# louislung/DAE_RNN_News_Recommendation

Hardware: NVIDIA H100
Metric: articles/sec (higher is better)
Workload: dtype f32

## Files before the change

dae_rnn_news_recommendation_b200/csrc/gemm_tc.cu:

```cuda
#include <cuda.h>
#include <cuda_bf16.h>
#include <type_traits>
#include "common.cuh"
#include "topk.cuh"

namespace dae {

constexpr int BLOCK_M = 128;
constexpr int BLOCK_K = 64;
constexpr int WGMMA_K = 16;
constexpr int kThreads = 384;
constexpr int kDecodeN = 128;

__device__ __forceinline__ uint32_t smem_u32(const void* p) { return (uint32_t)__cvta_generic_to_shared(p); }

__device__ __forceinline__ void mbar_init(uint64_t* bar, uint32_t count) {
  asm volatile("mbarrier.init.shared::cta.b64 [%0], %1;" ::"r"(smem_u32(bar)), "r"(count));
}
__device__ __forceinline__ void mbar_expect_tx(uint64_t* bar, uint32_t bytes) {
  asm volatile("mbarrier.arrive.expect_tx.shared::cta.b64 _, [%0], %1;" ::"r"(smem_u32(bar)), "r"(bytes) : "memory");
}
__device__ __forceinline__ void mbar_arrive(uint64_t* bar) {
  asm volatile("mbarrier.arrive.shared::cta.b64 _, [%0];" ::"r"(smem_u32(bar)) : "memory");
}
__device__ __forceinline__ bool mbar_try_wait(uint64_t* bar, uint32_t parity) {
  uint32_t ok;
  asm volatile(
      "{\n"
      ".reg .pred p;\n"
      "mbarrier.try_wait.parity.shared::cta.b64 p, [%1], %2;\n"
      "selp.u32 %0, 1, 0, p;\n"
      "}\n"
      : "=r"(ok)
      : "r"(smem_u32(bar)), "r"(parity)
      : "memory");
  return ok != 0;
}
__device__ __forceinline__ void mbar_wait(uint64_t* bar, uint32_t parity) {
  uint32_t spins = 0;
  while (!mbar_try_wait(bar, parity)) {
    if (++spins > 4096u) {
      __nanosleep(64);
      if (spins > (1u << 26)) __trap();
    }
  }
}
__device__ __forceinline__ void fence_barrier_init() { asm volatile("fence.mbarrier_init.release.cluster;" ::: "memory"); }

__device__ __forceinline__ void tma_load_2d(const CUtensorMap* map, uint64_t* bar, void* dst, int c0, int c1) {
  asm volatile(
      "cp.async.bulk.tensor.2d.shared::cluster.global.mbarrier::complete_tx::bytes [%0], [%1, {%3, %4}], [%2];" ::"r"(smem_u32(dst)),
      "l"(map), "r"(smem_u32(bar)), "r"(c0), "r"(c1)
      : "memory");
}
__device__ __forceinline__ uint32_t cluster_ctarank() { uint32_t r; asm volatile("mov.u32 %0, %%cluster_ctarank;" : "=r"(r)); return r; }
__device__ __forceinline__ void cluster_sync_all() {
  asm volatile("barrier.cluster.arrive.release.aligned;" ::: "memory");
  asm volatile("barrier.cluster.wait.acquire.aligned;" ::: "memory");
}
__device__ __forceinline__ void tma_load_2d_mc(const CUtensorMap* map, uint64_t* bar, void* dst, int c0, int c1, uint16_t cta_mask) {
  asm volatile(
      "cp.async.bulk.tensor.2d.shared::cluster.global.mbarrier::complete_tx::bytes.multicast::cluster [%0], [%1, {%3, %4}], [%2], %5;" ::"r"(
          smem_u32(dst)),
      "l"(map), "r"(smem_u32(bar)), "r"(c0), "r"(c1), "h"(cta_mask)
      : "memory");
}
__device__ __forceinline__ void mbar_arrive_cluster(uint64_t* bar, uint32_t rank) {
  uint32_t raddr;
  asm volatile("mapa.shared::cluster.u32 %0, %1, %2;" : "=r"(raddr) : "r"(smem_u32(bar)), "r"(rank));
  asm volatile("mbarrier.arrive.release.cluster.shared::cluster.b64 _, [%0];" ::"r"(raddr) : "memory");
}
__device__ __forceinline__ void mbar_wait_cluster(uint64_t* bar, uint32_t parity) {
  uint32_t spins = 0;
  for (;;) {
    uint32_t ok;
    asm volatile(
        "{\n"
        ".reg .pred p;\n"
        "mbarrier.try_wait.parity.acquire.cluster.shared::cta.b64 p, [%1], %2;\n"
        "selp.u32 %0, 1, 0, p;\n"
        "}\n"
        : "=r"(ok)
        : "r"(smem_u32(bar)), "r"(parity)
        : "memory");
    if (ok) return;
    if (++spins > 4096u) { __nanosleep(64); if (spins > (1u << 26)) __trap(); }
  }
}

__device__ __forceinline__ void prefetch_tmap(const CUtensorMap* map) {
  asm volatile("prefetch.tensormap [%0];" ::"l"(map) : "memory");
}
__device__ __forceinline__ void named_bar_sync(int id, int threads) { asm volatile("bar.sync %0, %1;" ::"r"(id), "r"(threads) : "memory"); }

__device__ __forceinline__ void wgmma_fence() { asm volatile("wgmma.fence.sync.aligned;" ::: "memory"); }
__device__ __forceinline__ void wgmma_commit() { asm volatile("wgmma.commit_group.sync.aligned;" ::: "memory"); }
template <int N>
__device__ __forceinline__ void wgmma_wait() { asm volatile("wgmma.wait_group.sync.aligned %0;" ::"n"(N) : "memory"); }

__device__ __forceinline__ uint64_t make_desc(uint32_t saddr, uint32_t lbo_bytes, uint32_t sbo_bytes, uint32_t layout = 1) {
  uint64_t d = 0;
  d |= (uint64_t)((saddr >> 4) & 0x3FFF);
  d |= (uint64_t)((lbo_bytes >> 4) & 0x3FFF) << 16;
  d |= (uint64_t)((sbo_bytes >> 4) & 0x3FFF) << 32;
  d |= (uint64_t)layout << 62;
  return d;
}


template <int TA, int TB>
__device__ __forceinline__ void wgmma_n128(float (&d)[64], uint64_t da, uint64_t db, uint32_t scale_d) {
  asm volatile(
      "{\n"
      ".reg .pred p;\n"
      "setp.ne.b32 p, %66, 0;\n"
      "wgmma.mma_async.sync.aligned.m64n128k16.f32.bf16.bf16 "
      "{%0, %1, %2, %3, %4, %5, %6, %7, %8, %9, %10, %11, %12, %13, %14, %15, %16, %17, %18, %19, %20, %21, %22, %23, %24, %25, %26, %27, %28, %29, %30, %31, %32, %33, %34, %35, %36, %37, %38, %39, %40, %41, %42, %43, %44, %45, %46, %47, %48, %49, %50, %51, %52, %53, %54, %55, %56, %57, %58, %59, %60, %61, %62, %63}, %64, %65, p, 1, 1, %67, %68;\n"
      "}\n"
      : "+f"(d[0]), "+f"(d[1]), "+f"(d[2]), "+f"(d[3]), "+f"(d[4]), "+f"(d[5]), "+f"(d[6]), "+f"(d[7]), "+f"(d[8]), "+f"(d[9]), "+f"(d[10]), "+f"(d[11]), "+f"(d[12]), "+f"(d[13]), "+f"(d[14]), "+f"(d[15]), "+f"(d[16]), "+f"(d[17]), "+f"(d[18]), "+f"(d[19]), "+f"(d[20]), "+f"(d[21]), "+f"(d[22]), "+f"(d[23]), "+f"(d[24]), "+f"(d[25]), "+f"(d[26]), "+f"(d[27]), "+f"(d[28]), "+f"(d[29]), "+f"(d[30]), "+f"(d[31]), "+f"(d[32]), "+f"(d[33]), "+f"(d[34]), "+f"(d[35]), "+f"(d[36]), "+f"(d[37]), "+f"(d[38]), "+f"(d[39]), "+f"(d[40]), "+f"(d[41]), "+f"(d[42]), "+f"(d[43]), "+f"(d[44]), "+f"(d[45]), "+f"(d[46]), "+f"(d[47]), "+f"(d[48]), "+f"(d[49]), "+f"(d[50]), "+f"(d[51]), "+f"(d[52]), "+f"(d[53]), "+f"(d[54]), "+f"(d[55]), "+f"(d[56]), "+f"(d[57]), "+f"(d[58]), "+f"(d[59]), "+f"(d[60]), "+f"(d[61]), "+f"(d[62]), "+f"(d[63])
      : "l"(da), "l"(db), "r"(scale_d), "n"(TA), "n"(TB));
}

template <int TA, int TB>
__device__ __forceinline__ void wgmma_n64(float (&d)[32], uint64_t da, uint64_t db, uint32_t scale_d) {
  asm volatile(
      "{\n"
      ".reg .pred p;\n"
      "setp.ne.b32 p, %34, 0;\n"
      "wgmma.mma_async.sync.aligned.m64n64k16.f32.bf16.bf16 "
      "{%0, %1, %2, %3, %4, %5, %6, %7, %8, %9, %10, %11, %12, %13, %14, %15, %16, %17, %18, %19, %20, %21, %22, %23, %24, %25, %26, %27, %28, %29, %30, %31}, %32, %33, p, 1, 1, %35, %36;\n"
      "}\n"
      : "+f"(d[0]), "+f"(d[1]), "+f"(d[2]), "+f"(d[3]), "+f"(d[4]), "+f"(d[5]), "+f"(d[6]), "+f"(d[7]), "+f"(d[8]), "+f"(d[9]), "+f"(d[10]), "+f"(d[11]), "+f"(d[12]), "+f"(d[13]), "+f"(d[14]), "+f"(d[15]), "+f"(d[16]), "+f"(d[17]), "+f"(d[18]), "+f"(d[19]), "+f"(d[20]), "+f"(d[21]), "+f"(d[22]), "+f"(d[23]), "+f"(d[24]), "+f"(d[25]), "+f"(d[26]), "+f"(d[27]), "+f"(d[28]), "+f"(d[29]), "+f"(d[30]), "+f"(d[31])
      : "l"(da), "l"(db), "r"(scale_d), "n"(TA), "n"(TB));
}

struct GemmParams {
  int M, N, K;
  int k_splits;
  int stream_k;
  int atomic;
  int a_mn, b_mn;
  int a_sym_kb;
  float alpha;
  float* C;
  int64_t ldc;
  int n_store;
  int special_col;
  float* special_out;
  const int64_t* indptr; const int32_t* indices; const float* values; const int32_t* rows;
  const float* bv; const float* weight; const double* stats;
  __nv_bfloat16* dz_hi; __nv_bfloat16* dz_lo; int64_t ld_dz;
  float* row_loss_part;
  const int32_t* tile_ptr;
};

struct Sched {
  int tiles_m, tiles, kb_total, kb_per_split, n_work, stream, w, n_cta;
  long long u, u_end;
  __device__ __forceinline__ void init(const GemmParams& p, int block_n, int pair = 0, int block_k = BLOCK_K) {
    const int cta = pair ? (int)(blockIdx.x >> 1) : (int)blockIdx.x;
    n_cta = pair ? (int)(gridDim.x >> 1) : (int)gridDim.x;
    tiles_m = (p.M + BLOCK_M - 1) / BLOCK_M;
    if (pair) tiles_m = (tiles_m + 1) / 2;
    tiles = tiles_m * ((p.N + block_n - 1) / block_n);
    kb_total = (p.K + block_k - 1) / block_k;
    stream = p.stream_k;
    kb_per_split = (kb_total + p.k_splits - 1) / p.k_splits;
    n_work = tiles * p.k_splits;
    w = cta;
    const long long U = (long long)tiles * kb_total;
    u = (long long)cta * U / n_cta;
    u_end = (long long)(cta + 1) * U / n_cta;
  }
  __device__ __forceinline__ bool next(int& mb, int& nb, int& kb0, int& kb1) {
    int tile;
    if (stream) {
      if (u >= u_end) return false;
      tile = (int)(u / kb_total);
      kb0 = (int)(u - (long long)tile * kb_total);
      const long long left = u_end - u;
      kb1 = (left < (long long)(kb_total - kb0)) ? kb0 + (int)left : kb_total;
      u += kb1 - kb0;
    } else {
      if (w >= n_work) return false;
      tile = w % tiles;
      kb0 = (w / tiles) * kb_per_split;
      kb1 = min(kb_total, kb0 + kb_per_split);
      w += n_cta;
    }
    mb = tile % tiles_m;
    nb = tile / tiles_m;
    return true;
  }
};

__device__ __forceinline__ uint32_t pack_bf16(float a, float b) {
  const __nv_bfloat162 v = __floats2bfloat162_rn(a, b);
  return *reinterpret_cast<const uint32_t*>(&v);
}
__device__ __forceinline__ float f_rcp(float x) { float r; asm("rcp.approx.ftz.f32 %0, %1;" : "=f"(r) : "f"(x)); return r; }
__device__ __forceinline__ float f_lg2(float x) { float r; asm("lg2.approx.ftz.f32 %0, %1;" : "=f"(r) : "f"(x)); return r; }
__device__ __forceinline__ float f_ex2(float x) { float r; asm("ex2.approx.ftz.f32 %0, %1;" : "=f"(r) : "f"(x)); return r; }
constexpr float kLog2e = 1.4426950408889634f;

template <int ACT>
__device__ __forceinline__ float act_fast(float z) {
  if (ACT == DAE_ACT_SIGMOID) return f_rcp(1.0f + f_ex2(-kLog2e * z));
  if (ACT == DAE_ACT_TANH) return 1.0f - 2.0f * f_rcp(1.0f + f_ex2(2.0f * kLog2e * z));
  return z;
}


__device__ __forceinline__ float select16(const uint32_t (&r)[16], int j) {
  uint32_t v = r[0];
#pragma unroll
  for (int k = 1; k < 16; ++k) v = (j == k) ? r[k] : v;
  return __uint_as_float(v);
}

template <int ACT, int LOSS>
__device__ __forceinline__ void decode_chunk_generic(const uint32_t (&r)[16], const float* __restrict__ bias, float sc, bool edge,
                                                     int n_lim, int nc, uint32_t (&hpk)[8], uint32_t (&lpk)[8], float& lsum) {
#pragma unroll
  for (int j2 = 0; j2 < 8; ++j2) {
    float dzp[2];
#pragma unroll
    for (int e = 0; e < 2; ++e) {
      const int j = 2 * j2 + e;
      const float z = __uint_as_float(r[j]) + bias[j];
      const float d = act_fast<ACT>(z);
      float dz, lt;
      if (LOSS == DAE_LOSS_CE) {
        const float omd = 1.0f - d;
        const float b = omd + kEps;
        lt = -f_lg2(b);
        dz = (ACT == DAE_ACT_SIGMOID) ? ((omd != 0.0f) ? sc * d : 0.0f) : sc * act_grad_from_y<ACT>(d) * f_rcp(b);
      } else {
        lt = d * d;
        dz = 2.0f * sc * d * act_grad_from_y<ACT>(d);
      }
      if (edge) { const bool in = (nc + j < n_lim); lt = in ? lt : 0.0f; dz = in ? dz : 0.0f; }
      lsum += lt;
      dzp[e] = dz;
    }
    const uint32_t hp = pack_bf16(dzp[0], dzp[1]);
    hpk[j2] = hp;
    lpk[j2] = pack_bf16(dzp[0] - __uint_as_float(hp << 16), dzp[1] - __uint_as_float(hp & 0xffff0000u));
  }
}

__device__ __forceinline__ bool decode_chunk_sigmoid_ce(const uint32_t (&r)[16], const float* __restrict__ biasc, float sc,
                                                        uint32_t (&hpk)[8], uint32_t (&lpk)[8], float& lsum) {
  bool ok = true;
#pragma unroll
  for (int g = 0; g < 4; ++g) {
    float t[4], a[4];
#pragma unroll
    for (int j = 0; j < 4; ++j) {
      t[j] = f_ex2(fmaf(__uint_as_float(r[4 * g + j]), kLog2e, biasc[4 * g + j]));
      a[j] = 1.0f + t[j];
    }
    const float p01 = a[0] * a[1], p23 = a[2] * a[3], P = p01 * p23;
    ok = ok && (P <= 22026.0f);
    const float Rs = f_rcp(P) * sc;
    lsum += f_lg2(P);
    const float r23 = Rs * p23, r01 = Rs * p01;
    const float dz0 = t[0] * (r23 * a[1]), dz1 = t[1] * (r23 * a[0]), dz2 = t[2] * (r01 * a[3]), dz3 = t[3] * (r01 * a[2]);
    const uint32_t h0 = pack_bf16(dz0, dz1), h1 = pack_bf16(dz2, dz3);
    hpk[2 * g] = h0; hpk[2 * g + 1] = h1;
    lpk[2 * g] = pack_bf16(dz0 - __uint_as_float(h0 << 16), dz1 - __uint_as_float(h0 & 0xffff0000u));
    lpk[2 * g + 1] = pack_bf16(dz2 - __uint_as_float(h1 << 16), dz3 - __uint_as_float(h1 & 0xffff0000u));
  }
  return ok;
}

template <int BLOCK_N, int TA, int TB, int BK = BLOCK_K>
__device__ __forceinline__ void mma_kblock(float (&acc)[BLOCK_N / 2], uint32_t sa_hi, uint32_t sa_lo, uint32_t sb_hi, uint32_t sb_lo,
                                           bool first) {
  static_assert(BK == 64 || BK == 32, "k-blocks are 32 or 64 wide");
  constexpr uint32_t kmaj_layout = BK == 64 ? 1u : 2u, kmaj_sbo = BK == 64 ? 1024u : 512u, mn_lbo = 64u * BK * 2u;
  constexpr uint32_t a_layout = TA ? 1u : kmaj_layout, b_layout = TB ? 1u : kmaj_layout;
  constexpr uint32_t a_sbo = TA ? 1024u : kmaj_sbo, b_sbo = TB ? 1024u : kmaj_sbo;
  constexpr uint32_t a_lbo = TA ? mn_lbo : 16u, b_lbo = TB ? mn_lbo : 16u;
  constexpr uint32_t a_step = TA ? 2048u : 32u, b_step = TB ? 2048u : 32u;
#pragma unroll
  for (int k = 0; k < BK / WGMMA_K; ++k) {
    const uint64_t da_hi = make_desc(sa_hi + k * a_step, a_lbo, a_sbo, a_layout), da_lo = make_desc(sa_lo + k * a_step, a_lbo, a_sbo, a_layout);
    const uint64_t db_hi = make_desc(sb_hi + k * b_step, b_lbo, b_sbo, b_layout), db_lo = make_desc(sb_lo + k * b_step, b_lbo, b_sbo, b_layout);
    const uint32_t sc = (first && k == 0) ? 0u : 1u;
    if constexpr (BLOCK_N == 128) {
      wgmma_n128<TA, TB>(acc, da_lo, db_hi, sc);
      wgmma_n128<TA, TB>(acc, da_hi, db_lo, 1u);
      wgmma_n128<TA, TB>(acc, da_hi, db_hi, 1u);
    } else {
      wgmma_n64<TA, TB>(acc, da_lo, db_hi, sc);
      wgmma_n64<TA, TB>(acc, da_hi, db_lo, 1u);
      wgmma_n64<TA, TB>(acc, da_hi, db_hi, 1u);
    }
  }
}

__device__ __forceinline__ void stage_ld16(const float* src, uint32_t (&r)[16]) {
#pragma unroll
  for (int q = 0; q < 4; ++q) {
    const float4 v = reinterpret_cast<const float4*>(src)[q];
    r[4 * q] = __float_as_uint(v.x); r[4 * q + 1] = __float_as_uint(v.y); r[4 * q + 2] = __float_as_uint(v.z); r[4 * q + 3] = __float_as_uint(v.w);
  }
}


template <int BLOCK_N, int STAGES, int PAIR, int BK = BLOCK_K, class SchedT>
__device__ __forceinline__ void tma_produce(const GemmParams& p, SchedT& sched, uint8_t* smem, uint64_t* full_bar, uint64_t* empty_bar,
                                            uint32_t crank, const CUtensorMap* tm_a_hi, const CUtensorMap* tm_a_lo,
                                            const CUtensorMap* tm_b_hi, const CUtensorMap* tm_b_lo, const CUtensorMap* tm_at_hi,
                                            const CUtensorMap* tm_at_lo) {
  constexpr int A_TILE = BLOCK_M * BK * 2;
  constexpr int B_TILE = BLOCK_N * BK * 2;
  constexpr int STAGE_BYTES = 2 * A_TILE + 2 * B_TILE;
  int stage = 0; uint32_t phase = 0;
  int mb, nb, kb0, kb1;
  while (sched.next(mb, nb, kb0, kb1)) {
    for (int kb = kb0; kb < kb1; ++kb) {
      if (PAIR) mbar_wait_cluster(&empty_bar[stage], phase ^ 1); else mbar_wait(&empty_bar[stage], phase ^ 1);
      uint8_t* sa_hi = smem + stage * STAGE_BYTES;
      uint8_t* sa_lo = sa_hi + A_TILE;
      uint8_t* sb_hi = sa_lo + A_TILE;
      uint8_t* sb_lo = sb_hi + B_TILE;
      const int mt = PAIR ? mb * 2 + (int)crank : mb;
      mbar_expect_tx(&full_bar[stage], STAGE_BYTES);
      if (p.a_sym_kb > 0 && kb >= p.a_sym_kb) {
#pragma unroll
        for (int j = 0; j < BLOCK_M / 64; ++j) {
          tma_load_2d(tm_at_hi, &full_bar[stage], sa_hi + j * (64 * BK * 2), mt * BLOCK_M + j * 64, (kb - p.a_sym_kb) * BK);
          tma_load_2d(tm_at_lo, &full_bar[stage], sa_lo + j * (64 * BK * 2), mt * BLOCK_M + j * 64, (kb - p.a_sym_kb) * BK);
        }
      } else if (!p.a_mn) {
        tma_load_2d(tm_a_hi, &full_bar[stage], sa_hi, kb * BK, mt * BLOCK_M);
        tma_load_2d(tm_a_lo, &full_bar[stage], sa_lo, kb * BK, mt * BLOCK_M);
      } else {
#pragma unroll
        for (int j = 0; j < BLOCK_M / 64; ++j) {
          tma_load_2d(tm_a_hi, &full_bar[stage], sa_hi + j * (64 * BK * 2), mt * BLOCK_M + j * 64, kb * BK);
          tma_load_2d(tm_a_lo, &full_bar[stage], sa_lo + j * (64 * BK * 2), mt * BLOCK_M + j * 64, kb * BK);
        }
      }
      const int kbb = (p.a_sym_kb > 0 && kb >= p.a_sym_kb) ? kb - p.a_sym_kb : kb;
      if (PAIR) {
        const int off = (int)crank * 8192, n_half = nb * BLOCK_N + (int)crank * 64;
        if (!p.b_mn) {
          tma_load_2d_mc(tm_b_hi, &full_bar[stage], sb_hi + off, kbb * BK, n_half, 0x3);
          tma_load_2d_mc(tm_b_lo, &full_bar[stage], sb_lo + off, kbb * BK, n_half, 0x3);
        } else {
          tma_load_2d_mc(tm_b_hi, &full_bar[stage], sb_hi + off, n_half, kbb * BK, 0x3);
          tma_load_2d_mc(tm_b_lo, &full_bar[stage], sb_lo + off, n_half, kbb * BK, 0x3);
        }
      } else if (!p.b_mn) {
        tma_load_2d(tm_b_hi, &full_bar[stage], sb_hi, kbb * BK, nb * BLOCK_N);
        tma_load_2d(tm_b_lo, &full_bar[stage], sb_lo, kbb * BK, nb * BLOCK_N);
      } else {
#pragma unroll
        for (int j = 0; j < BLOCK_N / 64; ++j) {
          tma_load_2d(tm_b_hi, &full_bar[stage], sb_hi + j * (64 * BK * 2), nb * BLOCK_N + j * 64, kbb * BK);
          tma_load_2d(tm_b_lo, &full_bar[stage], sb_lo + j * (64 * BK * 2), nb * BLOCK_N + j * 64, kbb * BK);
        }
      }
      if (++stage == STAGES) { stage = 0; phase ^= 1; }
    }
  }
}

template <int BLOCK_N, int STAGES, int PAIR, int MAJ, int BK = BLOCK_K>
__device__ __forceinline__ void mma_work_item(float (&acc)[BLOCK_N / 2], const GemmParams& p, uint8_t* smem, uint64_t* full_bar,
                                              uint64_t* empty_bar, int wg, int lane, uint32_t crank, int& stage, uint32_t& phase,
                                              int kb0, int kb1) {
  constexpr int A_TILE = BLOCK_M * BK * 2;
  constexpr int B_TILE = BLOCK_N * BK * 2;
  constexpr int STAGE_BYTES = 2 * A_TILE + 2 * B_TILE;
  auto release = [&](int s) {
    __syncwarp();
    if (lane == 0) { mbar_arrive(&empty_bar[s]); if (PAIR) mbar_arrive_cluster(&empty_bar[s], crank ^ 1u); }
  };
  int prev = -1;
  auto run_k = [&](auto ta, auto tb, int kb_begin, int kb_end) {
    for (int kb = kb_begin; kb < kb_end; ++kb) {
      mbar_wait(&full_bar[stage], phase);
      const uint32_t sa_hi = smem_u32(smem + stage * STAGE_BYTES) + wg * (64 * BK * 2);
      const uint32_t sa_lo = sa_hi + A_TILE;
      const uint32_t sb_hi = smem_u32(smem + stage * STAGE_BYTES) + 2 * A_TILE, sb_lo = sb_hi + B_TILE;
      wgmma_fence();
      mma_kblock<BLOCK_N, decltype(ta)::value, decltype(tb)::value, BK>(acc, sa_hi, sa_lo, sb_hi, sb_lo, kb == kb0);
      wgmma_commit();
      wgmma_wait<1>();
      if (prev >= 0) release(prev);
      prev = stage;
      if (++stage == STAGES) { stage = 0; phase ^= 1; }
    }
  };
  using K0 = std::integral_constant<int, 0>;
  using K1 = std::integral_constant<int, 1>;
  if constexpr ((MAJ & 4) != 0) {
    run_k(K0{}, K1{}, kb0, min(kb1, p.a_sym_kb));
    run_k(K1{}, K1{}, max(kb0, p.a_sym_kb), kb1);
  } else {
    run_k(std::integral_constant<int, MAJ & 1>{}, std::integral_constant<int, (MAJ >> 1) & 1>{}, kb0, kb1);
  }
  wgmma_wait<0>();
  if (prev >= 0) release(prev);
}

template <int BLOCK_N, int STAGES, int PAIR, int MAJ, int BK = BLOCK_K>
__global__ void __launch_bounds__(kThreads, 1) gemm_bf16x3_kernel(const __grid_constant__ CUtensorMap tm_a_hi,
                                                                   const __grid_constant__ CUtensorMap tm_a_lo,
                                                                   const __grid_constant__ CUtensorMap tm_b_hi,
                                                                   const __grid_constant__ CUtensorMap tm_b_lo,
                                                                   const __grid_constant__ CUtensorMap tm_at_hi,
                                                                   const __grid_constant__ CUtensorMap tm_at_lo,
                                                                   const GemmParams p) {
  static_assert(!PAIR || BLOCK_N == 128, "CTA pairs split the B tile into two 64-row halves");
  constexpr int STAGE_BYTES = 2 * BLOCK_M * BK * 2 + 2 * BLOCK_N * BK * 2;
  constexpr int SROW = BLOCK_N + 4;
  constexpr int kParts = 2;
  constexpr int HALF_N = BLOCK_N / kParts;
  extern __shared__ __align__(1024) uint8_t smem_raw[];
  uint8_t* smem = reinterpret_cast<uint8_t*>((reinterpret_cast<uintptr_t>(smem_raw) + 1023) & ~(uintptr_t)1023);
  float* stg = reinterpret_cast<float*>(smem + STAGES * STAGE_BYTES);
  __shared__ __align__(8) uint64_t full_bar[STAGES], empty_bar[STAGES];

  const int warp = threadIdx.x >> 5, lane = threadIdx.x & 31;
  Sched sched;
  sched.init(p, BLOCK_N, PAIR, BK);
  const uint32_t crank = PAIR ? cluster_ctarank() : 0u;

  if (warp == 0 && lane == 0) {
    prefetch_tmap(&tm_a_hi); prefetch_tmap(&tm_a_lo); prefetch_tmap(&tm_b_hi); prefetch_tmap(&tm_b_lo);
    if (p.a_sym_kb > 0) { prefetch_tmap(&tm_at_hi); prefetch_tmap(&tm_at_lo); }
  }
  if (warp == 1 && lane == 0) {
    for (int s = 0; s < STAGES; ++s) { mbar_init(&full_bar[s], 1); mbar_init(&empty_bar[s], PAIR ? 16 : 8); }
    fence_barrier_init();
  }
  if (PAIR) cluster_sync_all(); else __syncthreads();

  if (warp == 0) {
    if (lane == 0)
      tma_produce<BLOCK_N, STAGES, PAIR, BK>(p, sched, smem, full_bar, empty_bar, crank, &tm_a_hi, &tm_a_lo, &tm_b_hi, &tm_b_lo, &tm_at_hi,
                                         &tm_at_lo);
  } else if (warp >= 4) {
    const int wg = (warp >> 2) - 1;
    const int wi = warp & 3;
    const int quarter = wg * 2 + (wi & 1);
    const int half = wi >> 1;
    float acc[BLOCK_N / 2];
#pragma unroll
    for (int i = 0; i < BLOCK_N / 2; ++i) acc[i] = 0.0f;
    int stage = 0; uint32_t phase = 0;
    int mb, nb, kb0, kb1;
    while (sched.next(mb, nb, kb0, kb1)) {
      if (PAIR) mb = mb * 2 + (int)crank;
      mma_work_item<BLOCK_N, STAGES, PAIR, MAJ, BK>(acc, p, smem, full_bar, empty_bar, wg, lane, crank, stage, phase, kb0, kb1);

      named_bar_sync(1 + wg, 128);
      {
        const int r0 = wg * 64 + wi * 16 + (lane >> 2), c0 = 2 * (lane & 3);
#pragma unroll
        for (int j = 0; j < BLOCK_N / 8; ++j) {
          *reinterpret_cast<float2*>(&stg[r0 * SROW + 8 * j + c0]) = make_float2(acc[4 * j], acc[4 * j + 1]);
          *reinterpret_cast<float2*>(&stg[(r0 + 8) * SROW + 8 * j + c0]) = make_float2(acc[4 * j + 2], acc[4 * j + 3]);
        }
      }
      named_bar_sync(1 + wg, 128);
      const int n0 = nb * BLOCK_N + half * HALF_N;
      const float* tr = stg + (quarter * 32) * SROW + half * HALF_N;
      const int m_base = mb * BLOCK_M + quarter * 32;
      const bool vec_ok = ((p.ldc & 3) == 0) && ((reinterpret_cast<uintptr_t>(p.C) & 15) == 0);
#pragma unroll 1
      for (int c = 0; c < HALF_N / 16; ++c) {
        const int nc = n0 + c * 16;
        const bool interior = vec_ok && (m_base + 32 <= p.M) && (nc + 16 <= p.n_store) && (p.special_col < nc || p.special_col >= nc + 16);
        if (interior) {
          const int rsub = lane >> 2, c4 = (lane & 3) * 4;
          float* dst = p.C + (int64_t)(m_base + rsub) * p.ldc + nc + c4;
          const int64_t step = 8 * p.ldc;
#pragma unroll
          for (int i = 0; i < 4; ++i) {
            float4 v = *reinterpret_cast<const float4*>(&tr[(rsub + 8 * i) * SROW + c * 16 + c4]);
            v.x *= p.alpha; v.y *= p.alpha; v.z *= p.alpha; v.w *= p.alpha;
            if (p.atomic) atomicAdd(reinterpret_cast<float4*>(dst), v); else *reinterpret_cast<float4*>(dst) = v;
            dst += step;
          }
        } else {
          const int rsub = lane >> 4, csub = lane & 15;
          const int n = nc + csub;
          for (int i = 0; i < 16; ++i) {
            const int rr = 2 * i + rsub;
            const int mm = m_base + rr;
            const float v = p.alpha * tr[rr * SROW + c * 16 + csub];
            if (mm < p.M) {
              if (n == p.special_col) {
                if (p.atomic) atomicAdd(p.special_out + mm, v); else p.special_out[mm] = v;
              } else if (n < p.n_store) {
                float* dst = p.C + (int64_t)mm * p.ldc + n;
                if (p.atomic) atomicAdd(dst, v); else *dst = v;
              }
            }
          }
        }
      }
    }
  }

  if (PAIR) cluster_sync_all();
}

constexpr int kDecodeThreads = 640;
constexpr int kDecodeBK = 32;
constexpr int kDecodeStages = 4;
constexpr int kRegsProducer = 32, kRegsMma = 104, kRegsEpilogue = 120;
static_assert(128 * kRegsProducer + 256 * kRegsMma + 256 * kRegsEpilogue <= kDecodeThreads * 96, "register budget");

template <int R> __device__ __forceinline__ void regs_dec() { asm volatile("setmaxnreg.dec.sync.aligned.u32 %0;" ::"n"(R)); }
template <int R> __device__ __forceinline__ void regs_inc() { asm volatile("setmaxnreg.inc.sync.aligned.u32 %0;" ::"n"(R)); }

template <int ACT, int LOSS>
__global__ void __launch_bounds__(kDecodeThreads, 1) decode_fused_kernel(const __grid_constant__ CUtensorMap tm_a_hi,
                                                                         const __grid_constant__ CUtensorMap tm_a_lo,
                                                                         const __grid_constant__ CUtensorMap tm_b_hi,
                                                                         const __grid_constant__ CUtensorMap tm_b_lo,
                                                                         const GemmParams p) {
  constexpr int BLOCK_N = kDecodeN, STAGES = kDecodeStages, BK = kDecodeBK;
  constexpr int STAGE_BYTES = 2 * BLOCK_M * BK * 2 + 2 * BLOCK_N * BK * 2;
  constexpr int SROW = BLOCK_N + 4;
  constexpr int kParts = 2;
  constexpr int HALF_N = BLOCK_N / kParts;
  constexpr bool kFast = (ACT == DAE_ACT_SIGMOID) && (LOSS == DAE_LOSS_CE);
  extern __shared__ __align__(1024) uint8_t smem_raw[];
  uint8_t* smem = reinterpret_cast<uint8_t*>((reinterpret_cast<uintptr_t>(smem_raw) + 1023) & ~(uintptr_t)1023);
  float* stg = reinterpret_cast<float*>(smem + STAGES * STAGE_BYTES);
  __shared__ __align__(8) uint64_t full_bar[STAGES], empty_bar[STAGES], staged_bar[2], drained_bar[2];
  __shared__ float s_bias[2][BLOCK_N];
  __shared__ float s_biasc[kFast ? 2 : 1][kFast ? BLOCK_N : 1];
  __shared__ __align__(16) uint8_t s_stage[8][2][32][48];

  const int warp = threadIdx.x >> 5, lane = threadIdx.x & 31;
  const int role = warp >> 2;
  Sched sched;

  if (warp == 0 && lane == 0) { prefetch_tmap(&tm_a_hi); prefetch_tmap(&tm_a_lo); prefetch_tmap(&tm_b_hi); prefetch_tmap(&tm_b_lo); }
  if (warp == 1 && lane == 0) {
    for (int s = 0; s < STAGES; ++s) { mbar_init(&full_bar[s], 1); mbar_init(&empty_bar[s], 8); }
    for (int h = 0; h < 2; ++h) { mbar_init(&staged_bar[h], 4); mbar_init(&drained_bar[h], 4); }
    fence_barrier_init();
  }
  __syncthreads();

  if (role == 0) {
    regs_dec<kRegsProducer>();
    sched.init(p, BLOCK_N, 0, BK);
    if (warp == 0 && lane == 0)
      tma_produce<BLOCK_N, STAGES, 0, BK>(p, sched, smem, full_bar, empty_bar, 0u, &tm_a_hi, &tm_a_lo, &tm_b_hi, &tm_b_lo, &tm_a_hi, &tm_a_lo);
  } else if (role <= 2) {
    regs_inc<kRegsMma>();
    sched.init(p, BLOCK_N, 0, BK);
    const int h = role - 1;
    const int wi = warp & 3;
    float acc[BLOCK_N / 2];
#pragma unroll
    for (int i = 0; i < BLOCK_N / 2; ++i) acc[i] = 0.0f;
    int stage = 0; uint32_t phase = 0, tphase = 0;
    int mb, nb, kb0, kb1;
    while (sched.next(mb, nb, kb0, kb1)) {
      mma_work_item<BLOCK_N, STAGES, 0, 0, BK>(acc, p, smem, full_bar, empty_bar, h, lane, 0u, stage, phase, kb0, kb1);
      mbar_wait(&drained_bar[h], tphase ^ 1);
      const int r0 = h * 64 + wi * 16 + (lane >> 2), c0 = 2 * (lane & 3);
#pragma unroll
      for (int j = 0; j < BLOCK_N / 8; ++j) {
        *reinterpret_cast<float2*>(&stg[r0 * SROW + 8 * j + c0]) = make_float2(acc[4 * j], acc[4 * j + 1]);
        *reinterpret_cast<float2*>(&stg[(r0 + 8) * SROW + 8 * j + c0]) = make_float2(acc[4 * j + 2], acc[4 * j + 3]);
      }
      __syncwarp();
      if (lane == 0) mbar_arrive(&staged_bar[h]);
      tphase ^= 1;
    }
  } else {
    regs_inc<kRegsEpilogue>();
    sched.init(p, BLOCK_N, 0, BK);
    const int h = role - 3;
    const int ew = warp - 12;
    const int wi = warp & 3;
    const int quarter = h * 2 + (wi & 1);
    const int half = wi >> 1;
    const int row_in_tile = quarter * 32 + lane;
    const int tid = threadIdx.x - 128 * role;
    const int tiles_n = (p.N + BLOCK_N - 1) / BLOCK_N;
    uint8_t* stg_hi = reinterpret_cast<uint8_t*>(&s_stage[ew][0][0][0]);
    uint8_t* stg_lo = reinterpret_cast<uint8_t*>(&s_stage[ew][1][0][0]);
    const int rsub = lane >> 1, csub = lane & 1;
    uint32_t tphase = 0;
    int mb, nb, kb0, kb1;
    while (sched.next(mb, nb, kb0, kb1)) {
      const float* srow = stg + row_in_tile * SROW + half * HALF_N;
      const int m = mb * BLOCK_M + row_in_tile;
      const int n0 = nb * BLOCK_N + half * HALF_N;
      int64_t pc = 0, pe = 0;
      int c0 = 0x7fffffff, c1 = 0x7fffffff, c2 = 0x7fffffff;
      float v0 = 0.0f, v1 = 0.0f, v2 = 0.0f;
      float sc = 0.0f;
      if (m < p.M) {
        const int64_t row = p.rows ? (int64_t)p.rows[m] : (int64_t)m;
        const int64_t rbeg = p.indptr[row];
        const int32_t* tp = p.tile_ptr + (int64_t)m * (kParts * tiles_n + 1) + nb * kParts + half;
        pc = rbeg + tp[0]; pe = rbeg + tp[1];
        if (pc < pe) { c0 = p.indices[pc]; v0 = p.values[pc]; }
        if (pc + 1 < pe) { c1 = p.indices[pc + 1]; v1 = p.values[pc + 1]; }
        if (pc + 2 < pe) { c2 = p.indices[pc + 2]; v2 = p.values[pc + 2]; }
        sc = (p.weight ? p.weight[m] : 1.0f) / ((float)p.stats[DAE_STAT_SUM_W] + kEps);
      }
      named_bar_sync(1 + h, 128);
      {
        const float b = (nb * BLOCK_N + tid < p.N) ? p.bv[nb * BLOCK_N + tid] : 0.0f;
        s_bias[h][tid] = b;
        if (kFast) s_biasc[h][tid] = b * kLog2e;
      }
      mbar_wait(&staged_bar[h], tphase);
      named_bar_sync(1 + h, 128);
      const float inv_sc = (sc != 0.0f) ? 1.0f / sc : 0.0f;
      const bool edge = (n0 + HALF_N > p.N);
      float lsum = 0.0f;
      const int m_base = mb * BLOCK_M + quarter * 32;
      const int n_lim = edge ? p.N : 0x7fffffff;
#pragma unroll 1
      for (int c = 0; c < HALF_N / 16; ++c) {
        uint32_t r[16];
        stage_ld16(srow + c * 16, r);
        const int nc = n0 + c * 16;
        if (m < p.M) {
          const float* bias = &s_bias[h][half * HALF_N + c * 16];
          uint32_t hpk[8], lpk[8];
          bool fast_ok = false;
          if (kFast && !edge) {
            const float l0 = lsum;
            fast_ok = decode_chunk_sigmoid_ce(r, &s_biasc[h][half * HALF_N + c * 16], sc, hpk, lpk, lsum);
            if (!fast_ok) { lsum = l0; decode_chunk_generic<ACT, LOSS>(r, bias, sc, edge, n_lim, nc, hpk, lpk, lsum); }
          } else {
            decode_chunk_generic<ACT, LOSS>(r, bias, sc, edge, n_lim, nc, hpk, lpk, lsum);
          }
          uint4* sh = reinterpret_cast<uint4*>(stg_hi + lane * 48);
          uint4* sl = reinterpret_cast<uint4*>(stg_lo + lane * 48);
          sh[0] = make_uint4(hpk[0], hpk[1], hpk[2], hpk[3]); sh[1] = make_uint4(hpk[4], hpk[5], hpk[6], hpk[7]);
          sl[0] = make_uint4(lpk[0], lpk[1], lpk[2], lpk[3]); sl[1] = make_uint4(lpk[4], lpk[5], lpk[6], lpk[7]);
          while (c0 < nc + 16) {
            const float x = v0;
            const int j = c0 - nc;
            __nv_bfloat16* ph = reinterpret_cast<__nv_bfloat16*>(stg_hi + lane * 48) + j;
            __nv_bfloat16* pl = reinterpret_cast<__nv_bfloat16*>(stg_lo + lane * 48) + j;
            float d;
            if (kFast && fast_ok && sc != 0.0f) d = (__bfloat162float(*ph) + __bfloat162float(*pl)) * inv_sc;
            else d = act_fast<ACT>(select16(r, j) + bias[j]);
            const float gp = act_grad_from_y<ACT>(d);
            float dz;
            if (LOSS == DAE_LOSS_CE) {
              const float a = d + kEps, b = (1.0f - d) + kEps;
              const float la = f_lg2(a), lb = f_lg2(b);
              lsum += lb - (x * la + (1.0f - x) * lb);
              dz = sc * gp * ((1.0f - x) * f_rcp(b) - x * f_rcp(a));
            } else {
              const float e2 = x - d;
              lsum += e2 * e2 - d * d;
              dz = -2.0f * sc * e2 * gp;
            }
            const __nv_bfloat16 hb = __float2bfloat16_rn(dz);
            *ph = hb;
            *pl = __float2bfloat16_rn(dz - __bfloat162float(hb));
            ++pc;
            c0 = c1; v0 = v1; c1 = c2; v1 = v2;
            c2 = 0x7fffffff;
            if (pc + 2 < pe) { c2 = p.indices[pc + 2]; v2 = p.values[pc + 2]; }
          }
        }
        __syncwarp();
        if (nc < p.ld_dz) {
#pragma unroll
          for (int i = 0; i < 2; ++i) {
            const int rr = rsub + 16 * i;
            if (m_base + rr < p.M) {
              const int64_t off = (int64_t)(m_base + rr) * p.ld_dz + nc + csub * 8;
              *reinterpret_cast<uint4*>(p.dz_hi + off) = *reinterpret_cast<const uint4*>(stg_hi + rr * 48 + csub * 16);
              *reinterpret_cast<uint4*>(p.dz_lo + off) = *reinterpret_cast<const uint4*>(stg_lo + rr * 48 + csub * 16);
            }
          }
        }
        __syncwarp();
      }
      if (lane == 0) mbar_arrive(&drained_bar[h]);
      tphase ^= 1;
      if (m < p.M) atomicAdd(p.row_loss_part + m, (LOSS == DAE_LOSS_CE) ? lsum * 0.6931471805599453f : lsum);
    }
  }
}

constexpr int kTopkMaxK = 32;
constexpr int kTopkMaxSplits = 32;
constexpr int kTopkMinTiles = 4;
constexpr int kTopkBK = 64;
constexpr int kTopkStages = 2;

struct TopkParams {
  GemmParams g;
  int k, splits;
  int exclude;
  int64_t diag_offset;
  float* ws_val; int32_t* ws_idx;
};

struct TopkSched {
  int tiles_n, splits, kb_total, n_work, n_cta, w;
  int mb, split, t, t_end;
  bool first, last;
  __device__ __forceinline__ void init(const TopkParams& tp, int block_n, int block_k) {
    const int tiles_m = (tp.g.M + BLOCK_M - 1) / BLOCK_M;
    tiles_n = (tp.g.N + block_n - 1) / block_n;
    splits = tp.splits;
    kb_total = (tp.g.K + block_k - 1) / block_k;
    n_work = tiles_m * splits;
    n_cta = (int)gridDim.x;
    w = (int)blockIdx.x - n_cta;
    mb = split = t = t_end = 0;
    first = last = false;
  }
  __device__ __forceinline__ bool next(int& mb_, int& nb, int& kb0, int& kb1) {
    first = false;
    if (t >= t_end) {
      w += n_cta;
      if (w >= n_work) return false;
      mb = w / splits;
      split = w - mb * splits;
      t = split * tiles_n / splits;
      t_end = (split + 1) * tiles_n / splits;
      first = true;
    }
    mb_ = mb; nb = t; kb0 = 0; kb1 = kb_total;
    last = (++t == t_end);
    return true;
  }
};

template <int KMAX>
__device__ __forceinline__ void topk_offer(float (&sv)[KMAX], int (&si)[KMAX], float& thr, int k, float v, int col, int n_lim,
                                           int excl) {
  if (!(v > thr) || col >= n_lim || col == excl) return;
#pragma unroll
  for (int j = KMAX - 1; j >= 0; --j) {
    const bool up = (j > 0) && (v > sv[j > 0 ? j - 1 : 0]);
    const bool here = v > sv[j];
    si[j] = up ? si[j > 0 ? j - 1 : 0] : (here ? col : si[j]);
    sv[j] = up ? sv[j > 0 ? j - 1 : 0] : (here ? v : sv[j]);
  }
  float t = sv[0];
#pragma unroll
  for (int j = 1; j < KMAX; ++j)
    asm("{\n.reg .pred q;\nsetp.eq.s32 q, %1, %2;\nselp.f32 %0, %3, %0, q;\n}\n" : "+f"(t) : "r"(j), "r"(k - 1), "f"(sv[j]));
  thr = t;
}

template <int KMAX>
__global__ void __launch_bounds__(kDecodeThreads, 1) topk_kernel(const __grid_constant__ CUtensorMap tm_a_hi,
                                                                 const __grid_constant__ CUtensorMap tm_a_lo,
                                                                 const __grid_constant__ CUtensorMap tm_b_hi,
                                                                 const __grid_constant__ CUtensorMap tm_b_lo,
                                                                 const TopkParams tp) {
  constexpr int BLOCK_N = kDecodeN, STAGES = kTopkStages, BK = kTopkBK;
  constexpr int STAGE_BYTES = 2 * BLOCK_M * BK * 2 + 2 * BLOCK_N * BK * 2;
  constexpr int SROW = BLOCK_N + 4;
  constexpr int HALF_N = BLOCK_N / 2;
  const GemmParams& p = tp.g;
  extern __shared__ __align__(1024) uint8_t smem_raw[];
  uint8_t* smem = reinterpret_cast<uint8_t*>((reinterpret_cast<uintptr_t>(smem_raw) + 1023) & ~(uintptr_t)1023);
  float* stg = reinterpret_cast<float*>(smem + STAGES * STAGE_BYTES);
  __shared__ __align__(8) uint64_t full_bar[STAGES], empty_bar[STAGES], staged_bar[2], drained_bar[2];

  const int warp = threadIdx.x >> 5, lane = threadIdx.x & 31;
  const int role = warp >> 2;
  TopkSched sched;

  if (warp == 0 && lane == 0) { prefetch_tmap(&tm_a_hi); prefetch_tmap(&tm_a_lo); prefetch_tmap(&tm_b_hi); prefetch_tmap(&tm_b_lo); }
  if (warp == 1 && lane == 0) {
    for (int s = 0; s < STAGES; ++s) { mbar_init(&full_bar[s], 1); mbar_init(&empty_bar[s], 8); }
    for (int h = 0; h < 2; ++h) { mbar_init(&staged_bar[h], 4); mbar_init(&drained_bar[h], 4); }
    fence_barrier_init();
  }
  __syncthreads();

  if (role == 0) {
    regs_dec<kRegsProducer>();
    sched.init(tp, BLOCK_N, BK);
    if (warp == 0 && lane == 0)
      tma_produce<BLOCK_N, STAGES, 0, BK>(p, sched, smem, full_bar, empty_bar, 0u, &tm_a_hi, &tm_a_lo, &tm_b_hi, &tm_b_lo, &tm_a_hi, &tm_a_lo);
  } else if (role <= 2) {
    regs_inc<kRegsMma>();
    sched.init(tp, BLOCK_N, BK);
    const int h = role - 1;
    const int wi = warp & 3;
    float acc[BLOCK_N / 2];
#pragma unroll
    for (int i = 0; i < BLOCK_N / 2; ++i) acc[i] = 0.0f;
    int stage = 0; uint32_t phase = 0, tphase = 0;
    int mb, nb, kb0, kb1;
    while (sched.next(mb, nb, kb0, kb1)) {
      mma_work_item<BLOCK_N, STAGES, 0, 0, BK>(acc, p, smem, full_bar, empty_bar, h, lane, 0u, stage, phase, kb0, kb1);
      mbar_wait(&drained_bar[h], tphase ^ 1);
      const int r0 = h * 64 + wi * 16 + (lane >> 2), c0 = 2 * (lane & 3);
#pragma unroll
      for (int j = 0; j < BLOCK_N / 8; ++j) {
        *reinterpret_cast<float2*>(&stg[r0 * SROW + 8 * j + c0]) = make_float2(acc[4 * j], acc[4 * j + 1]);
        *reinterpret_cast<float2*>(&stg[(r0 + 8) * SROW + 8 * j + c0]) = make_float2(acc[4 * j + 2], acc[4 * j + 3]);
      }
      __syncwarp();
      if (lane == 0) mbar_arrive(&staged_bar[h]);
      tphase ^= 1;
    }
  } else {
    regs_inc<kRegsEpilogue>();
    sched.init(tp, BLOCK_N, BK);
    const int h = role - 3;
    const int wi = warp & 3;
    const int quarter = h * 2 + (wi & 1);
    const int half = wi >> 1;
    const int row_in_tile = quarter * 32 + lane;
    const int k = tp.k;
    const float* srow = stg + row_in_tile * SROW + half * HALF_N;
    float sv[KMAX];
    int si[KMAX];
    float thr = neg_inf();
    int m = 0, excl = -1;
    uint32_t tphase = 0;
    int mb, nb, kb0, kb1;
    while (sched.next(mb, nb, kb0, kb1)) {
      if (sched.first) {
#pragma unroll
        for (int j = 0; j < KMAX; ++j) { sv[j] = neg_inf(); si[j] = -1; }
        thr = neg_inf();
        m = mb * BLOCK_M + row_in_tile;
        const int64_t e = (int64_t)m + tp.diag_offset;
        excl = (tp.exclude && e >= 0 && e < p.N) ? (int)e : -1;
      }
      const int n0 = nb * BLOCK_N + half * HALF_N;
      mbar_wait(&staged_bar[h], tphase);
      if (m < p.M) {
#pragma unroll 1
        for (int c = 0; c < HALF_N; c += 4) {
          const float4 v = *reinterpret_cast<const float4*>(srow + c);
          if (fmaxf(fmaxf(v.x, v.y), fmaxf(v.z, v.w)) > thr) {
            topk_offer<KMAX>(sv, si, thr, k, v.x, n0 + c, p.N, excl);
            topk_offer<KMAX>(sv, si, thr, k, v.y, n0 + c + 1, p.N, excl);
            topk_offer<KMAX>(sv, si, thr, k, v.z, n0 + c + 2, p.N, excl);
            topk_offer<KMAX>(sv, si, thr, k, v.w, n0 + c + 3, p.N, excl);
          }
        }
      }
      __syncwarp();
      if (lane == 0) mbar_arrive(&drained_bar[h]);
      tphase ^= 1;
      if (sched.last && m < p.M) {
        const int64_t base = ((int64_t)m * (2 * sched.splits) + 2 * sched.split + half) * k;
#pragma unroll
        for (int j = 0; j < KMAX; ++j)
          if (j < k) { tp.ws_val[base + j] = sv[j]; tp.ws_idx[base + j] = si[j]; }
      }
    }
  }
}

__global__ void decode_tile_ptr_kernel(const int64_t* __restrict__ indptr, const int32_t* __restrict__ indices,
                                       const int32_t* __restrict__ rows, int M, int n_half_tiles, int half_n,
                                       int32_t* __restrict__ tile_ptr) {
  const int t = blockIdx.x * blockDim.x + threadIdx.x;
  const int m = blockIdx.y;
  if (t > n_half_tiles || m >= M) return;
  const int64_t row = rows ? (int64_t)rows[m] : (int64_t)m;
  const int64_t b = indptr[row], e = indptr[row + 1];
  const int target = t * half_n;
  int64_t lo = b, hi = e;
  while (lo < hi) { const int64_t mid = (lo + hi) >> 1; if (indices[mid] < target) lo = mid + 1; else hi = mid; }
  tile_ptr[(int64_t)m * (n_half_tiles + 1) + t] = (int32_t)(lo - b);
}

__global__ void split_bf16_kernel(const float* __restrict__ src, int rows, int cols, int64_t ld_src, __nv_bfloat16* __restrict__ hi,
                                  __nv_bfloat16* __restrict__ lo, int64_t ld_dst, int ones_col, float scale) {
  const int64_t total = (int64_t)rows * ld_dst;
  for (int64_t i = (int64_t)blockIdx.x * blockDim.x + threadIdx.x; i < total; i += (int64_t)gridDim.x * blockDim.x) {
    const int64_t r = i / ld_dst;
    const int c = (int)(i - r * ld_dst);
    float v = (c < cols) ? src[r * ld_src + c] * scale : 0.0f;
    if (c == ones_col) v = 1.0f;
    const __nv_bfloat16 h = __float2bfloat16_rn(v);
    hi[i] = h;
    lo[i] = __float2bfloat16_rn(v - __bfloat162float(h));
  }
}

__global__ void sym_split_kernel(const float* __restrict__ G, int B, int64_t ldg, float alpha, __nv_bfloat16* __restrict__ hi,
                                 __nv_bfloat16* __restrict__ lo, int64_t ld) {
  __shared__ float t[32][33];
  const int bx = blockIdx.x * 32, by = blockIdx.y * 32;
  const int tx = threadIdx.x, ty = threadIdx.y;
  for (int j = ty; j < 32; j += 8) {
    const int r = bx + j, c = by + tx;
    t[j][tx] = (r < B && c < B) ? G[(int64_t)r * ldg + c] : 0.0f;
  }
  __syncthreads();
  for (int j = ty; j < 32; j += 8) {
    const int r = by + j, c = bx + tx;
    if (r < B && c < ld) {
      float v = 0.0f;
      if (c < B) v = alpha * (G[(int64_t)r * ldg + c] + t[tx][j]);
      const __nv_bfloat16 h = __float2bfloat16_rn(v);
      hi[(int64_t)r * ld + c] = h;
      lo[(int64_t)r * ld + c] = __float2bfloat16_rn(v - __bfloat162float(h));
    }
  }
}

typedef CUresult (*PFN_encodeTiled)(CUtensorMap*, CUtensorMapDataType, cuuint32_t, void*, const cuuint64_t*, const cuuint64_t*,
                                    const cuuint32_t*, const cuuint32_t*, CUtensorMapInterleave, CUtensorMapSwizzle,
                                    CUtensorMapL2promotion, CUtensorMapFloatOOBfill);

static PFN_encodeTiled get_encode() {
  static PFN_encodeTiled fn = nullptr;
  if (!fn) {
    void* sym = nullptr;
    cudaDriverEntryPointQueryResult q;
    if (cudaGetDriverEntryPoint("cuTensorMapEncodeTiled", &sym, cudaEnableDefault, &q) == cudaSuccess && q == cudaDriverEntryPointSuccess)
      fn = reinterpret_cast<PFN_encodeTiled>(sym);
  }
  return fn;
}

static int make_map(CUtensorMap* m, const void* base, uint64_t inner, uint64_t outer, uint64_t ld, uint32_t box_outer,
                    uint32_t box_inner = 64) {
  PFN_encodeTiled enc = get_encode();
  if (!enc) { set_error("cuTensorMapEncodeTiled entry point not found"); return DAE_ERR_CUDA; }
  cuuint64_t dims[2] = {inner, outer};
  cuuint64_t strides[1] = {ld * 2};
  cuuint32_t box[2] = {box_inner, box_outer};
  cuuint32_t estr[2] = {1, 1};
  CUresult r = enc(m, CU_TENSOR_MAP_DATA_TYPE_BFLOAT16, 2, const_cast<void*>(base), dims, strides, box, estr,
                   CU_TENSOR_MAP_INTERLEAVE_NONE, box_inner == 64 ? CU_TENSOR_MAP_SWIZZLE_128B : CU_TENSOR_MAP_SWIZZLE_64B,
                   CU_TENSOR_MAP_L2_PROMOTION_L2_256B,
                   CU_TENSOR_MAP_FLOAT_OOB_FILL_NONE);
  if (r != CUDA_SUCCESS) { set_error("cuTensorMapEncodeTiled failed (%d): inner=%llu outer=%llu ld=%llu", (int)r,
                                     (unsigned long long)inner, (unsigned long long)outer, (unsigned long long)ld); return DAE_ERR_CUDA; }
  return DAE_OK;
}

struct Operand { const void* hi; const void* lo; int64_t ld; int mn_major; };

template <typename Kern>
static int ensure_smem_attr(Kern kern, int smem, bool (&done)[64]) {
  int dev = 0;
  DAE_CUDA(cudaGetDevice(&dev));
  if (dev < 0 || dev >= 64 || !done[dev]) {
    DAE_CUDA(cudaFuncSetAttribute(kern, cudaFuncAttributeMaxDynamicSharedMemorySize, smem));
    if (dev >= 0 && dev < 64) done[dev] = true;
  }
  return DAE_OK;
}


static int g_pair_mode = -1;
static int g_lean = 0;

template <int BLOCK_N, int STAGES, int PAIR, int MAJ, int BK = BLOCK_K>
static int launch_gemm_maj(const Operand& A, const Operand& B, GemmParams p, cudaStream_t st) {
  CUtensorMap ta_hi, ta_lo, tb_hi, tb_lo;
  int rc;
  constexpr int B_ROWS = PAIR ? BLOCK_N / 2 : BLOCK_N;
  if (!A.mn_major) {
    const uint64_t a_cols = p.a_sym_kb > 0 ? (uint64_t)p.M : (uint64_t)p.K;
    if ((rc = make_map(&ta_hi, A.hi, a_cols, p.M, A.ld, BLOCK_M, BK))) return rc;
    if ((rc = make_map(&ta_lo, A.lo, a_cols, p.M, A.ld, BLOCK_M, BK))) return rc;
  } else {
    if ((rc = make_map(&ta_hi, A.hi, p.M, p.K, A.ld, BK))) return rc;
    if ((rc = make_map(&ta_lo, A.lo, p.M, p.K, A.ld, BK))) return rc;
  }
  if (!B.mn_major) {
    if ((rc = make_map(&tb_hi, B.hi, p.K, p.N, B.ld, B_ROWS, BK))) return rc;
    if ((rc = make_map(&tb_lo, B.lo, p.K, p.N, B.ld, B_ROWS, BK))) return rc;
  } else {
    const uint64_t b_rows = p.a_sym_kb > 0 ? (uint64_t)p.M : (uint64_t)p.K;
    if ((rc = make_map(&tb_hi, B.hi, p.N, b_rows, B.ld, BK))) return rc;
    if ((rc = make_map(&tb_lo, B.lo, p.N, b_rows, B.ld, BK))) return rc;
  }
  p.a_mn = A.mn_major; p.b_mn = B.mn_major;
  CUtensorMap tat_hi = ta_hi, tat_lo = ta_lo;
  if (p.a_sym_kb > 0) {
    if (PAIR || A.mn_major) { set_error("dae_gemm_sym_bf16x3: unsupported configuration"); return DAE_ERR_UNSUPPORTED; }
    if ((rc = make_map(&tat_hi, A.hi, p.M, p.M, A.ld, 64))) return rc;
    if ((rc = make_map(&tat_lo, A.lo, p.M, p.M, A.ld, 64))) return rc;
  }
  constexpr int smem = STAGES * (2 * BLOCK_M * BK * 2 + 2 * BLOCK_N * BK * 2) + BLOCK_M * (BLOCK_N + 4) * 4 + 1024;
  int tiles_m = (p.M + BLOCK_M - 1) / BLOCK_M;
  if (PAIR) tiles_m = (tiles_m + 1) / 2;
  const int tiles_n = (p.N + BLOCK_N - 1) / BLOCK_N;
  const int kblocks = (p.K + BK - 1) / BK;
  auto kern = gemm_bf16x3_kernel<BLOCK_N, STAGES, PAIR, MAJ, BK>;
  static bool attr_done[64] = {false};
  if ((rc = ensure_smem_attr(kern, smem, attr_done))) return rc;
  const int slots = PAIR ? sm_count() / 2 : sm_count();
  int n;
  if (p.stream_k) {
    const long long units = (long long)tiles_m * tiles_n * kblocks;
    long long g = units / (6 * BLOCK_K / BK);
    if (g < 1) g = 1;
    n = (int)(g < slots ? g : slots);
  } else {
    const int items = tiles_m * tiles_n * p.k_splits;
    n = items < slots ? items : slots;
  }
  if (!PAIR) {
    kern<<<n, kThreads, smem, st>>>(ta_hi, ta_lo, tb_hi, tb_lo, tat_hi, tat_lo, p);
  } else {
    cudaLaunchConfig_t cfg{};
    cfg.gridDim = dim3(2 * n); cfg.blockDim = dim3(kThreads); cfg.dynamicSmemBytes = smem; cfg.stream = st;
    cudaLaunchAttribute at[1];
    at[0].id = cudaLaunchAttributeClusterDimension;
    at[0].val.clusterDim.x = 2; at[0].val.clusterDim.y = 1; at[0].val.clusterDim.z = 1;
    cfg.attrs = at; cfg.numAttrs = 1;
    DAE_CUDA(cudaLaunchKernelEx(&cfg, kern, ta_hi, ta_lo, tb_hi, tb_lo, tat_hi, tat_lo, p));
  }
  return DAE_OK;
}

template <int BLOCK_N, int STAGES, int PAIR, int BK = BLOCK_K>
static int launch_gemm(const Operand& A, const Operand& B, GemmParams p, cudaStream_t st) {
  if (!A.mn_major && !B.mn_major) return launch_gemm_maj<BLOCK_N, STAGES, PAIR, 0, BK>(A, B, p, st);
  if (A.mn_major && !B.mn_major) return launch_gemm_maj<BLOCK_N, STAGES, PAIR, 1, BK>(A, B, p, st);
  if (!A.mn_major) return launch_gemm_maj<BLOCK_N, STAGES, PAIR, 2, BK>(A, B, p, st);
  return launch_gemm_maj<BLOCK_N, STAGES, PAIR, 3, BK>(A, B, p, st);
}

template <int ACT, int LOSS>
static int launch_decode(const Operand& A, const Operand& B, const GemmParams& p, cudaStream_t st) {
  CUtensorMap ta_hi, ta_lo, tb_hi, tb_lo;
  int rc;
  if ((rc = make_map(&ta_hi, A.hi, p.K, p.M, A.ld, BLOCK_M, kDecodeBK))) return rc;
  if ((rc = make_map(&ta_lo, A.lo, p.K, p.M, A.ld, BLOCK_M, kDecodeBK))) return rc;
  if ((rc = make_map(&tb_hi, B.hi, p.K, p.N, B.ld, kDecodeN, kDecodeBK))) return rc;
  if ((rc = make_map(&tb_lo, B.lo, p.K, p.N, B.ld, kDecodeN, kDecodeBK))) return rc;
  constexpr int smem = kDecodeStages * (2 * BLOCK_M * kDecodeBK * 2 + 2 * kDecodeN * kDecodeBK * 2) + BLOCK_M * (kDecodeN + 4) * 4 + 1024;
  auto kern = decode_fused_kernel<ACT, LOSS>;
  static bool attr_done[64] = {false};
  if ((rc = ensure_smem_attr(kern, smem, attr_done))) return rc;
  const int tiles = ((p.M + BLOCK_M - 1) / BLOCK_M) * ((p.N + kDecodeN - 1) / kDecodeN);
  const int n = tiles < sm_count() ? tiles : sm_count();
  kern<<<n, kDecodeThreads, smem, st>>>(ta_hi, ta_lo, tb_hi, tb_lo, p);
  return DAE_OK;
}

template <int KMAX>
static int launch_topk(const Operand& A, const Operand& B, const TopkParams& tp, cudaStream_t st) {
  CUtensorMap ta_hi, ta_lo, tb_hi, tb_lo;
  int rc;
  const GemmParams& p = tp.g;
  if ((rc = make_map(&ta_hi, A.hi, p.K, p.M, A.ld, BLOCK_M, kTopkBK))) return rc;
  if ((rc = make_map(&ta_lo, A.lo, p.K, p.M, A.ld, BLOCK_M, kTopkBK))) return rc;
  if ((rc = make_map(&tb_hi, B.hi, p.K, p.N, B.ld, kDecodeN, kTopkBK))) return rc;
  if ((rc = make_map(&tb_lo, B.lo, p.K, p.N, B.ld, kDecodeN, kTopkBK))) return rc;
  constexpr int smem = kTopkStages * (2 * BLOCK_M * kTopkBK * 2 + 2 * kDecodeN * kTopkBK * 2) + BLOCK_M * (kDecodeN + 4) * 4 + 1024;
  auto kern = topk_kernel<KMAX>;
  static bool attr_done[64] = {false};
  if ((rc = ensure_smem_attr(kern, smem, attr_done))) return rc;
  const int items = ((p.M + BLOCK_M - 1) / BLOCK_M) * tp.splits;
  const int n = items < sm_count() ? items : sm_count();
  kern<<<n, kDecodeThreads, smem, st>>>(ta_hi, ta_lo, tb_hi, tb_lo, tp);
  return DAE_OK;
}

static int topk_splits(int n_query, int n_corpus, int requested) {
  const int tiles_m = (n_query + BLOCK_M - 1) / BLOCK_M, tiles_n = (n_corpus + kDecodeN - 1) / kDecodeN;
  int s = requested;
  if (s <= 0) {
    s = (sm_count() + tiles_m - 1) / tiles_m;
    const int by_len = tiles_n / kTopkMinTiles;
    if (s > by_len) s = by_len;
  }
  if (s > tiles_n) s = tiles_n;
  if (s > kTopkMaxSplits) s = kTopkMaxSplits;
  return s < 1 ? 1 : s;
}

static int64_t topk_workspace_bytes(int n_query, int k, int splits) {
  return (int64_t)n_query * 2 * splits * k * (int64_t)(sizeof(float) + sizeof(int32_t));
}

static bool use_pair() { return g_pair_mode == 1 && !g_lean; }

}

using namespace dae;

extern "C" int dae_split_bf16(const float* src, int32_t rows, int32_t cols, int64_t ld_src, void* hi, void* lo, int64_t ld_dst,
                              int32_t ones_col, float scale, void* stream) {
  DAE_REQUIRE(src && hi && lo && rows > 0 && cols > 0 && ld_src >= cols && ld_dst >= cols, "dae_split_bf16: bad arguments");
  const int64_t total = (int64_t)rows * ld_dst;
  const int cap = sm_count() * 16;
  const int blocks = (int)((total + 255) / 256 < cap ? (total + 255) / 256 : cap);
  split_bf16_kernel<<<blocks, 256, 0, (cudaStream_t)stream>>>(src, rows, cols, ld_src, (__nv_bfloat16*)hi, (__nv_bfloat16*)lo, ld_dst,
                                                              ones_col, scale);
  DAE_CHECK_LAUNCH("dae_split_bf16");
  return DAE_OK;
}

extern "C" int dae_sym_split_bf16(const float* G, int32_t B, int64_t ldg, float alpha, void* hi, void* lo, int64_t ld, void* stream) {
  DAE_REQUIRE(G && hi && lo && B > 0 && ldg >= B && ld >= B, "dae_sym_split_bf16: bad arguments");
  dim3 grid((unsigned)((ld + 31) / 32), (B + 31) / 32), block(32, 8);
  sym_split_kernel<<<grid, block, 0, (cudaStream_t)stream>>>(G, B, ldg, alpha, (__nv_bfloat16*)hi, (__nv_bfloat16*)lo, ld);
  DAE_CHECK_LAUNCH("dae_sym_split_bf16");
  return DAE_OK;
}

extern "C" int dae_gemm_config(int32_t pair_mode, int32_t lean) {
  dae::g_pair_mode = pair_mode < 0 ? -1 : (pair_mode ? 1 : 0);
  dae::g_lean = lean ? 1 : 0;
  return DAE_OK;
}

extern "C" int dae_gemm_bf16x3(int32_t M, int32_t N, int32_t K, float alpha, const void* a_hi, const void* a_lo, int64_t lda,
                               int32_t a_mn_major, const void* b_hi, const void* b_lo, int64_t ldb, int32_t b_mn_major, float* C,
                               int64_t ldc, int32_t n_store, int32_t special_col, float* special_out, int32_t k_splits,
                               int32_t accumulate, void* stream) {
  DAE_REQUIRE(a_hi && a_lo && b_hi && b_lo && C && M > 0 && N > 0 && K > 0, "dae_gemm_bf16x3: bad arguments");
  DAE_REQUIRE(lda % 8 == 0 && ldb % 8 == 0, "dae_gemm_bf16x3: operand leading dimensions must be multiples of 8 (TMA 16-byte strides)");
  DAE_REQUIRE(((uintptr_t)a_hi | (uintptr_t)a_lo | (uintptr_t)b_hi | (uintptr_t)b_lo) % 16 == 0, "dae_gemm_bf16x3: operands must be 16-byte aligned");
  cudaStream_t st = (cudaStream_t)stream;
  if (n_store <= 0 || n_store > N) n_store = N;
  const int kblocks = (K + BLOCK_K - 1) / BLOCK_K;
  const int tm = (M + 127) / 128, tn128 = (N + 127) / 128, tn64 = (N + 63) / 64;
  const int sms = sm_count();
  int stream_k = 0;
  if (k_splits < 0) {
    const int t = tm * tn128;
    stream_k = (t % sms == 0) ? 0 : 1;
    k_splits = 1;
  }
  if (k_splits < 1) k_splits = 1;
  if (k_splits > kblocks) k_splits = kblocks;
  {
    const int per = (kblocks + k_splits - 1) / k_splits;
    k_splits = (kblocks + per - 1) / per;
  }
  const bool partial = (k_splits > 1) || stream_k;
  if (partial && !accumulate) {
    DAE_CUDA(cudaMemset2DAsync(C, ldc * sizeof(float), 0, (size_t)n_store * sizeof(float), M, st));
    if (special_col >= 0 && special_out) DAE_CUDA(cudaMemsetAsync(special_out, 0, sizeof(float) * M, st));
  }
  GemmParams p{};
  p.M = M; p.N = N; p.K = K; p.k_splits = k_splits; p.stream_k = stream_k; p.atomic = (partial || accumulate) ? 1 : 0; p.alpha = alpha;
  p.C = C; p.ldc = ldc; p.n_store = n_store;
  p.special_col = (special_out ? special_col : -1); p.special_out = special_out;
  Operand A{a_hi, a_lo, lda, a_mn_major}, B{b_hi, b_lo, ldb, b_mn_major};
  int rc;
  const int tiles128 = tm * tn128 * k_splits, tiles64 = tm * tn64 * k_splits;
  const float cost128 = 2.0f * (float)((tiles128 + sms - 1) / sms), cost64 = 1.1f * (float)((tiles64 + sms - 1) / sms);
  if (g_lean) rc = launch_gemm<64, 2, 0>(A, B, p, st);
  else if (use_pair()) rc = launch_gemm<128, 2, 1>(A, B, p, st);
  else if (stream_k) rc = launch_gemm<128, 4, 0, 32>(A, B, p, st);
  else if (!stream_k && cost64 < cost128) rc = launch_gemm<64, 3, 0>(A, B, p, st);
  else rc = launch_gemm<128, 2, 0>(A, B, p, st);
  if (rc) return rc;
  DAE_CHECK_LAUNCH("dae_gemm_bf16x3");
  return DAE_OK;
}

extern "C" int dae_gemm_sym_bf16x3(int32_t M, int32_t N, float alpha, const void* g_hi, const void* g_lo, int64_t ldg, const void* b_hi,
                                   const void* b_lo, int64_t ldb, float* C, int64_t ldc, int32_t accumulate, void* stream) {
  DAE_REQUIRE(g_hi && g_lo && b_hi && b_lo && C && M > 0 && N > 0, "dae_gemm_sym_bf16x3: bad arguments");
  DAE_REQUIRE(ldg % 8 == 0 && ldb % 8 == 0 && ldg >= M && ldb >= N, "dae_gemm_sym_bf16x3: leading dimensions must be multiples of 8 and cover the matrices");
  DAE_REQUIRE(((uintptr_t)g_hi | (uintptr_t)g_lo | (uintptr_t)b_hi | (uintptr_t)b_lo) % 16 == 0, "dae_gemm_sym_bf16x3: operands must be 16-byte aligned");
  GemmParams p{};
  const int kb_half = (M + BLOCK_K - 1) / BLOCK_K;
  p.M = M; p.N = N; p.K = 2 * kb_half * BLOCK_K; p.k_splits = 1; p.stream_k = 1; p.atomic = 1; p.alpha = alpha;
  p.C = C; p.ldc = ldc; p.n_store = N; p.special_col = -1; p.special_out = nullptr; p.a_sym_kb = kb_half;
  if (!accumulate) DAE_CUDA(cudaMemset2DAsync(C, ldc * sizeof(float), 0, (size_t)N * sizeof(float), M, (cudaStream_t)stream));
  Operand A{g_hi, g_lo, ldg, 0}, B{b_hi, b_lo, ldb, 1};
  int rc = launch_gemm_maj<128, 2, 0, 6>(A, B, p, (cudaStream_t)stream);
  if (rc) return rc;
  DAE_CHECK_LAUNCH("dae_gemm_sym_bf16x3");
  return DAE_OK;
}

extern "C" int dae_decode_prepare(int32_t Brows, int32_t F, const int64_t* indptr, const int32_t* indices, const int32_t* rows,
                                  float* row_loss_part, int32_t* tile_ptr, void* stream) {
  DAE_REQUIRE(Brows > 0 && F > 0 && indptr && indices && row_loss_part && tile_ptr, "dae_decode_prepare: bad arguments");
  cudaStream_t st = (cudaStream_t)stream;
  DAE_CUDA(cudaMemsetAsync(row_loss_part, 0, sizeof(float) * Brows, st));
  const int n_half = 2 * ((F + kDecodeN - 1) / kDecodeN);
  dim3 grid((n_half + 1 + 127) / 128, Brows);
  decode_tile_ptr_kernel<<<grid, 128, 0, st>>>(indptr, indices, rows, Brows, n_half, kDecodeN / 2, tile_ptr);
  DAE_CHECK_LAUNCH("dae_decode_prepare");
  return DAE_OK;
}

extern "C" int dae_decode_fused_bf16x3(int32_t Brows, int32_t F, int32_t K, const void* e_hi, const void* e_lo, int64_t lde,
                                       const void* w_hi, const void* w_lo, int64_t ldw, const int64_t* indptr, const int32_t* indices,
                                       const float* values, const int32_t* rows, const float* bv, int32_t dec_act, int32_t loss_func,
                                       const float* weight, const double* stats, void* dz_hi, void* dz_lo, int64_t ld_dz,
                                       float* row_loss_part, int32_t* tile_ptr, int32_t prepared, void* stream) {
  DAE_REQUIRE(e_hi && e_lo && w_hi && w_lo && indptr && indices && values && bv && stats && dz_hi && dz_lo && row_loss_part && tile_ptr,
              "dae_decode_fused_bf16x3: null pointer");
  DAE_REQUIRE(loss_func == DAE_LOSS_CE || loss_func == DAE_LOSS_MSE, "dae_decode_fused_bf16x3: cosine loss uses the unfused path");
  DAE_REQUIRE(lde % 8 == 0 && ldw % 8 == 0 && ld_dz % 32 == 0 && ld_dz >= F, "dae_decode_fused_bf16x3: bad leading dimensions");
  cudaStream_t st = (cudaStream_t)stream;
  GemmParams p{};
  p.M = Brows; p.N = F; p.K = K; p.k_splits = 1; p.alpha = 1.0f; p.special_col = -1;
  p.indptr = indptr; p.indices = indices; p.values = values; p.rows = rows; p.bv = bv; p.weight = weight; p.stats = stats;
  p.dz_hi = (__nv_bfloat16*)dz_hi; p.dz_lo = (__nv_bfloat16*)dz_lo; p.ld_dz = ld_dz; p.row_loss_part = row_loss_part;
  p.tile_ptr = tile_ptr;
  if (!prepared) {
    int rc0 = dae_decode_prepare(Brows, F, indptr, indices, rows, row_loss_part, tile_ptr, stream);
    if (rc0) return rc0;
  }
  Operand A{e_hi, e_lo, lde, 0}, B{w_hi, w_lo, ldw, 0};
  int rc = 0;
#define DAE_DEC(ACT, LOSS) rc = launch_decode<ACT, LOSS>(A, B, p, st)
  if (loss_func == DAE_LOSS_CE) {
    if (dec_act == DAE_ACT_SIGMOID) DAE_DEC(DAE_ACT_SIGMOID, DAE_LOSS_CE);
    else if (dec_act == DAE_ACT_TANH) DAE_DEC(DAE_ACT_TANH, DAE_LOSS_CE);
    else DAE_DEC(DAE_ACT_NONE, DAE_LOSS_CE);
  } else {
    if (dec_act == DAE_ACT_SIGMOID) DAE_DEC(DAE_ACT_SIGMOID, DAE_LOSS_MSE);
    else if (dec_act == DAE_ACT_TANH) DAE_DEC(DAE_ACT_TANH, DAE_LOSS_MSE);
    else DAE_DEC(DAE_ACT_NONE, DAE_LOSS_MSE);
  }
#undef DAE_DEC
  if (rc) return rc;
  DAE_CHECK_LAUNCH("dae_decode_fused_bf16x3");
  return DAE_OK;
}

extern "C" int dae_similarity_topk_workspace(int32_t n_query, int32_t n_corpus, int32_t k, int32_t splits, int64_t* bytes) {
  DAE_REQUIRE(bytes && n_query > 0 && n_corpus > 0, "dae_similarity_topk_workspace: bad arguments");
  DAE_REQUIRE(k >= 1 && k <= kTopkMaxK, "dae_similarity_topk_workspace: k = %d is outside the supported range 1 <= k <= %d", k, kTopkMaxK);
  *bytes = topk_workspace_bytes(n_query, k, topk_splits(n_query, n_corpus, splits));
  return DAE_OK;
}

extern "C" int dae_similarity_topk_bf16x3(int32_t n_query, int32_t n_corpus, int32_t dim, const void* q_hi, const void* q_lo, int64_t ldq,
                                          const void* c_hi, const void* c_lo, int64_t ldc, int32_t k, int64_t diag_offset, int32_t exclude,
                                          int32_t splits, void* workspace, int64_t workspace_bytes, int32_t* idx_out, float* val_out,
                                          void* stream) {
  DAE_REQUIRE(q_hi && q_lo && c_hi && c_lo && workspace && idx_out && val_out, "dae_similarity_topk_bf16x3: null pointer");
  DAE_REQUIRE(n_query > 0 && n_corpus > 0 && dim > 0, "dae_similarity_topk_bf16x3: bad sizes");
  DAE_REQUIRE(k >= 1 && k <= kTopkMaxK, "dae_similarity_topk_bf16x3: k = %d is outside the supported range 1 <= k <= %d", k, kTopkMaxK);
  DAE_REQUIRE(ldq >= dim && ldc >= dim && ldq % 8 == 0 && ldc % 8 == 0,
              "dae_similarity_topk_bf16x3: leading dimensions must cover dim and be multiples of 8 (TMA 16-byte strides)");
  DAE_REQUIRE(((uintptr_t)q_hi | (uintptr_t)q_lo | (uintptr_t)c_hi | (uintptr_t)c_lo | (uintptr_t)workspace) % 16 == 0,
              "dae_similarity_topk_bf16x3: operands and workspace must be 16-byte aligned");
  const int s = topk_splits(n_query, n_corpus, splits);
  const int64_t need = topk_workspace_bytes(n_query, k, s);
  DAE_REQUIRE(workspace_bytes >= need, "dae_similarity_topk_bf16x3: workspace of %lld bytes, %lld needed (dae_similarity_topk_workspace)",
              (long long)workspace_bytes, (long long)need);
  cudaStream_t st = (cudaStream_t)stream;
  TopkParams tp{};
  tp.g.M = n_query; tp.g.N = n_corpus; tp.g.K = dim; tp.g.k_splits = 1; tp.g.alpha = 1.0f; tp.g.special_col = -1;
  tp.k = k; tp.splits = s; tp.exclude = exclude ? 1 : 0; tp.diag_offset = diag_offset;
  tp.ws_val = reinterpret_cast<float*>(workspace);
  tp.ws_idx = reinterpret_cast<int32_t*>(reinterpret_cast<float*>(workspace) + (int64_t)n_query * 2 * s * k);
  Operand A{q_hi, q_lo, ldq, 0}, B{c_hi, c_lo, ldc, 0};
  int rc = (k <= 16) ? launch_topk<16>(A, B, tp, st) : launch_topk<32>(A, B, tp, st);
  if (rc) return rc;
  DAE_CHECK_LAUNCH("dae_similarity_topk_bf16x3");
  topk_merge_kernel<<<(n_query + 7) / 8, 256, 0, st>>>(tp.ws_val, tp.ws_idx, n_query, 2 * s, k, idx_out, val_out);
  DAE_CHECK_LAUNCH("dae_similarity_topk_bf16x3 (merge)");
  return DAE_OK;
}
```

Before: 2.294 million.

## Transpose fused decode GEMM with 160-wide batch tiles and simplified warp roles

The fused decode kernel now computes the transposed product, with features on the M side and batch rows on the N side, using m64n160k16 wgmma tiles. Warp roles drop from 20 warps with setmaxnreg rebalancing to 14 warps: 8 MMA warps, 5 epilogue warps and 1 TMA producer. Staging moves to a swizzled, column-major shared buffer that is reused in place for the bf16 outputs. This aims for better tensor-core tile shape and fewer barrier and staging round-trips, but it changes tile_ptr semantics, shrinks epilogue parallelism, and leaves one epilogue thread per batch row serially scanning 128 features.

After: 2.340 million, median of 6. 2.0% higher.

```diff
diff --git a/dae_rnn_news_recommendation_b200/csrc/gemm_tc.cu b/dae_rnn_news_recommendation_b200/csrc/gemm_tc.cu
--- a/dae_rnn_news_recommendation_b200/csrc/gemm_tc.cu
+++ b/dae_rnn_news_recommendation_b200/csrc/gemm_tc.cu
@@ -10,7 +10,6 @@
 constexpr int BLOCK_K = 64;
 constexpr int WGMMA_K = 16;
 constexpr int kThreads = 384;
-constexpr int kDecodeN = 128;
 
 __device__ __forceinline__ uint32_t smem_u32(const void* p) { return (uint32_t)__cvta_generic_to_shared(p); }
 
@@ -118,6 +117,19 @@
       "{%0, %1, %2, %3, %4, %5, %6, %7, %8, %9, %10, %11, %12, %13, %14, %15, %16, %17, %18, %19, %20, %21, %22, %23, %24, %25, %26, %27, %28, %29, %30, %31, %32, %33, %34, %35, %36, %37, %38, %39, %40, %41, %42, %43, %44, %45, %46, %47, %48, %49, %50, %51, %52, %53, %54, %55, %56, %57, %58, %59, %60, %61, %62, %63}, %64, %65, p, 1, 1, %67, %68;\n"
       "}\n"
       : "+f"(d[0]), "+f"(d[1]), "+f"(d[2]), "+f"(d[3]), "+f"(d[4]), "+f"(d[5]), "+f"(d[6]), "+f"(d[7]), "+f"(d[8]), "+f"(d[9]), "+f"(d[10]), "+f"(d[11]), "+f"(d[12]), "+f"(d[13]), "+f"(d[14]), "+f"(d[15]), "+f"(d[16]), "+f"(d[17]), "+f"(d[18]), "+f"(d[19]), "+f"(d[20]), "+f"(d[21]), "+f"(d[22]), "+f"(d[23]), "+f"(d[24]), "+f"(d[25]), "+f"(d[26]), "+f"(d[27]), "+f"(d[28]), "+f"(d[29]), "+f"(d[30]), "+f"(d[31]), "+f"(d[32]), "+f"(d[33]), "+f"(d[34]), "+f"(d[35]), "+f"(d[36]), "+f"(d[37]), "+f"(d[38]), "+f"(d[39]), "+f"(d[40]), "+f"(d[41]), "+f"(d[42]), "+f"(d[43]), "+f"(d[44]), "+f"(d[45]), "+f"(d[46]), "+f"(d[47]), "+f"(d[48]), "+f"(d[49]), "+f"(d[50]), "+f"(d[51]), "+f"(d[52]), "+f"(d[53]), "+f"(d[54]), "+f"(d[55]), "+f"(d[56]), "+f"(d[57]), "+f"(d[58]), "+f"(d[59]), "+f"(d[60]), "+f"(d[61]), "+f"(d[62]), "+f"(d[63])
+      : "l"(da), "l"(db), "r"(scale_d), "n"(TA), "n"(TB));
+}
+
+template <int TA, int TB>
+__device__ __forceinline__ void wgmma_n160(float (&d)[80], uint64_t da, uint64_t db, uint32_t scale_d) {
+  asm volatile(
+      "{\n"
+      ".reg .pred p;\n"
+      "setp.ne.b32 p, %82, 0;\n"
+      "wgmma.mma_async.sync.aligned.m64n160k16.f32.bf16.bf16 "
+      "{%0, %1, %2, %3, %4, %5, %6, %7, %8, %9, %10, %11, %12, %13, %14, %15, %16, %17, %18, %19, %20, %21, %22, %23, %24, %25, %26, %27, %28, %29, %30, %31, %32, %33, %34, %35, %36, %37, %38, %39, %40, %41, %42, %43, %44, %45, %46, %47, %48, %49, %50, %51, %52, %53, %54, %55, %56, %57, %58, %59, %60, %61, %62, %63, %64, %65, %66, %67, %68, %69, %70, %71, %72, %73, %74, %75, %76, %77, %78, %79}, %80, %81, p, 1, 1, %83, %84;\n"
+      "}\n"
+      : "+f"(d[0]), "+f"(d[1]), "+f"(d[2]), "+f"(d[3]), "+f"(d[4]), "+f"(d[5]), "+f"(d[6]), "+f"(d[7]), "+f"(d[8]), "+f"(d[9]), "+f"(d[10]), "+f"(d[11]), "+f"(d[12]), "+f"(d[13]), "+f"(d[14]), "+f"(d[15]), "+f"(d[16]), "+f"(d[17]), "+f"(d[18]), "+f"(d[19]), "+f"(d[20]), "+f"(d[21]), "+f"(d[22]), "+f"(d[23]), "+f"(d[24]), "+f"(d[25]), "+f"(d[26]), "+f"(d[27]), "+f"(d[28]), "+f"(d[29]), "+f"(d[30]), "+f"(d[31]), "+f"(d[32]), "+f"(d[33]), "+f"(d[34]), "+f"(d[35]), "+f"(d[36]), "+f"(d[37]), "+f"(d[38]), "+f"(d[39]), "+f"(d[40]), "+f"(d[41]), "+f"(d[42]), "+f"(d[43]), "+f"(d[44]), "+f"(d[45]), "+f"(d[46]), "+f"(d[47]), "+f"(d[48]), "+f"(d[49]), "+f"(d[50]), "+f"(d[51]), "+f"(d[52]), "+f"(d[53]), "+f"(d[54]), "+f"(d[55]), "+f"(d[56]), "+f"(d[57]), "+f"(d[58]), "+f"(d[59]), "+f"(d[60]), "+f"(d[61]), "+f"(d[62]), "+f"(d[63]), "+f"(d[64]), "+f"(d[65]), "+f"(d[66]), "+f"(d[67]), "+f"(d[68]), "+f"(d[69]), "+f"(d[70]), "+f"(d[71]), "+f"(d[72]), "+f"(d[73]), "+f"(d[74]), "+f"(d[75]), "+f"(d[76]), "+f"(d[77]), "+f"(d[78]), "+f"(d[79])
       : "l"(da), "l"(db), "r"(scale_d), "n"(TA), "n"(TB));
 }
 
@@ -216,6 +228,22 @@
 #pragma unroll
   for (int k = 1; k < 16; ++k) v = (j == k) ? r[k] : v;
   return __uint_as_float(v);
+}
+
+__device__ __forceinline__ uint32_t sel_if_eq(uint32_t v, int a, int b, uint32_t x) {
+  asm("{\n.reg .pred q;\nsetp.eq.s32 q, %1, %2;\nselp.b32 %0, %3, %0, q;\n}\n" : "+r"(v) : "r"(a), "r"(b), "r"(x));
+  return v;
+}
+__device__ __forceinline__ float bf16_get16(const uint32_t (&w)[8], int j) {
+  uint32_t v = w[0];
+#pragma unroll
+  for (int k = 1; k < 8; ++k) v = sel_if_eq(v, j >> 1, k, w[k]);
+  return __uint_as_float((j & 1) ? (v & 0xffff0000u) : (v << 16));
+}
+__device__ __forceinline__ void bf16_set16(uint32_t (&w)[8], int j, uint32_t bits) {
+  const int sh = (j & 1) * 16;
+#pragma unroll
+  for (int k = 0; k < 8; ++k) w[k] = sel_if_eq(w[k], j >> 1, k, (w[k] & ~(0xffffu << sh)) | (bits << sh));
 }
 
 template <int ACT, int LOSS>
@@ -288,7 +316,11 @@
     const uint64_t da_hi = make_desc(sa_hi + k * a_step, a_lbo, a_sbo, a_layout), da_lo = make_desc(sa_lo + k * a_step, a_lbo, a_sbo, a_layout);
     const uint64_t db_hi = make_desc(sb_hi + k * b_step, b_lbo, b_sbo, b_layout), db_lo = make_desc(sb_lo + k * b_step, b_lbo, b_sbo, b_layout);
     const uint32_t sc = (first && k == 0) ? 0u : 1u;
-    if constexpr (BLOCK_N == 128) {
+    if constexpr (BLOCK_N == 160) {
+      wgmma_n160<TA, TB>(acc, da_hi, db_lo, sc);
+      wgmma_n160<TA, TB>(acc, da_lo, db_hi, 1u);
+      wgmma_n160<TA, TB>(acc, da_hi, db_hi, 1u);
+    } else if constexpr (BLOCK_N == 128) {
       wgmma_n128<TA, TB>(acc, da_lo, db_hi, sc);
       wgmma_n128<TA, TB>(acc, da_hi, db_lo, 1u);
       wgmma_n128<TA, TB>(acc, da_hi, db_hi, 1u);
@@ -300,10 +332,10 @@
   }
 }
 
-__device__ __forceinline__ void stage_ld16(const float* src, uint32_t (&r)[16]) {
+__device__ __forceinline__ void stage_ld16(const float* row, int g0, int swz, uint32_t (&r)[16]) {
 #pragma unroll
   for (int q = 0; q < 4; ++q) {
-    const float4 v = reinterpret_cast<const float4*>(src)[q];
+    const float4 v = reinterpret_cast<const float4*>(row)[(g0 + q) ^ swz];
     r[4 * q] = __float_as_uint(v.x); r[4 * q + 1] = __float_as_uint(v.y); r[4 * q + 2] = __float_as_uint(v.z); r[4 * q + 3] = __float_as_uint(v.w);
   }
 }
@@ -512,14 +544,55 @@
   if (PAIR) cluster_sync_all();
 }
 
-constexpr int kDecodeThreads = 640;
+constexpr int kDecodeThreads = 448;
+constexpr int kDecodeN = 160;
 constexpr int kDecodeBK = 32;
 constexpr int kDecodeStages = 4;
-constexpr int kRegsProducer = 32, kRegsMma = 104, kRegsEpilogue = 120;
-static_assert(128 * kRegsProducer + 256 * kRegsMma + 256 * kRegsEpilogue <= kDecodeThreads * 96, "register budget");
-
-template <int R> __device__ __forceinline__ void regs_dec() { asm volatile("setmaxnreg.dec.sync.aligned.u32 %0;" ::"n"(R)); }
-template <int R> __device__ __forceinline__ void regs_inc() { asm volatile("setmaxnreg.inc.sync.aligned.u32 %0;" ::"n"(R)); }
+
+struct DecodeSched {
+  int w, tiles_n, tiles, kb_total;
+  __device__ __forceinline__ void init(const GemmParams& p) {
+    tiles_n = (p.N + kDecodeN - 1) / kDecodeN;
+    tiles = ((p.M + BLOCK_M - 1) / BLOCK_M) * tiles_n;
+    kb_total = (p.K + kDecodeBK - 1) / kDecodeBK;
+    w = (int)blockIdx.x;
+  }
+  __device__ __forceinline__ bool next(int& mb, int& nb, int& kb0, int& kb1) {
+    if (w >= tiles) return false;
+    mb = w / tiles_n; nb = w - mb * tiles_n;
+    kb0 = 0; kb1 = kb_total;
+    w += (int)gridDim.x;
+    return true;
+  }
+};
+
+struct DecodeRow {
+  int64_t pc, pe;
+  int c0, c1, c2;
+  float v0, v1, v2;
+  float sc;
+  __device__ __forceinline__ void open(const GemmParams& p, int m, int mb) {
+    pc = pe = 0;
+    c0 = c1 = c2 = 0x7fffffff;
+    v0 = v1 = v2 = 0.0f;
+    sc = 0.0f;
+    if (m >= p.N) return;
+    const int64_t row = p.rows ? (int64_t)p.rows[m] : (int64_t)m;
+    const int64_t rbeg = p.indptr[row];
+    const int32_t* tp = p.tile_ptr + (int64_t)m * (2 * ((p.M + BLOCK_M - 1) / BLOCK_M) + 1) + 2 * mb;
+    pc = rbeg + tp[0]; pe = rbeg + tp[2];
+    if (pc < pe) { c0 = p.indices[pc]; v0 = p.values[pc]; }
+    if (pc + 1 < pe) { c1 = p.indices[pc + 1]; v1 = p.values[pc + 1]; }
+    if (pc + 2 < pe) { c2 = p.indices[pc + 2]; v2 = p.values[pc + 2]; }
+    sc = (p.weight ? p.weight[m] : 1.0f) / ((float)p.stats[DAE_STAT_SUM_W] + kEps);
+  }
+  __device__ __forceinline__ void advance(const GemmParams& p) {
+    ++pc;
+    c0 = c1; v0 = v1; c1 = c2; v1 = v2;
+    c2 = 0x7fffffff;
+    if (pc + 2 < pe) { c2 = p.indices[pc + 2]; v2 = p.values[pc + 2]; }
+  }
+};
 
 template <int ACT, int LOSS>
 __global__ void __launch_bounds__(kDecodeThreads, 1) decode_fused_kernel(const __grid_constant__ CUtensorMap tm_a_hi,
@@ -529,132 +602,99 @@
                                                                          const GemmParams p) {
   constexpr int BLOCK_N = kDecodeN, STAGES = kDecodeStages, BK = kDecodeBK;
   constexpr int STAGE_BYTES = 2 * BLOCK_M * BK * 2 + 2 * BLOCK_N * BK * 2;
-  constexpr int SROW = BLOCK_N + 4;
-  constexpr int kParts = 2;
-  constexpr int HALF_N = BLOCK_N / kParts;
   constexpr bool kFast = (ACT == DAE_ACT_SIGMOID) && (LOSS == DAE_LOSS_CE);
   extern __shared__ __align__(1024) uint8_t smem_raw[];
   uint8_t* smem = reinterpret_cast<uint8_t*>((reinterpret_cast<uintptr_t>(smem_raw) + 1023) & ~(uintptr_t)1023);
   float* stg = reinterpret_cast<float*>(smem + STAGES * STAGE_BYTES);
-  __shared__ __align__(8) uint64_t full_bar[STAGES], empty_bar[STAGES], staged_bar[2], drained_bar[2];
-  __shared__ float s_bias[2][BLOCK_N];
-  __shared__ float s_biasc[kFast ? 2 : 1][kFast ? BLOCK_N : 1];
-  __shared__ __align__(16) uint8_t s_stage[8][2][32][48];
+  __shared__ __align__(8) uint64_t full_bar[STAGES], empty_bar[STAGES], staged_bar, drained_bar;
+  __shared__ float s_bias[BLOCK_M];
+  __shared__ float s_biasc[kFast ? BLOCK_M : 1];
 
   const int warp = threadIdx.x >> 5, lane = threadIdx.x & 31;
-  const int role = warp >> 2;
-  Sched sched;
-
-  if (warp == 0 && lane == 0) { prefetch_tmap(&tm_a_hi); prefetch_tmap(&tm_a_lo); prefetch_tmap(&tm_b_hi); prefetch_tmap(&tm_b_lo); }
-  if (warp == 1 && lane == 0) {
+  DecodeSched sched;
+  sched.init(p);
+
+  if (warp == 13 && lane == 0) { prefetch_tmap(&tm_a_hi); prefetch_tmap(&tm_a_lo); prefetch_tmap(&tm_b_hi); prefetch_tmap(&tm_b_lo); }
+  if (warp == 0 && lane == 0) {
     for (int s = 0; s < STAGES; ++s) { mbar_init(&full_bar[s], 1); mbar_init(&empty_bar[s], 8); }
-    for (int h = 0; h < 2; ++h) { mbar_init(&staged_bar[h], 4); mbar_init(&drained_bar[h], 4); }
+    mbar_init(&staged_bar, 8);
+    mbar_init(&drained_bar, 5);
     fence_barrier_init();
   }
   __syncthreads();
 
-  if (role == 0) {
-    regs_dec<kRegsProducer>();
-    sched.init(p, BLOCK_N, 0, BK);
-    if (warp == 0 && lane == 0)
+  if (warp == 13) {
+    if (lane == 0)
       tma_produce<BLOCK_N, STAGES, 0, BK>(p, sched, smem, full_bar, empty_bar, 0u, &tm_a_hi, &tm_a_lo, &tm_b_hi, &tm_b_lo, &tm_a_hi, &tm_a_lo);
-  } else if (role <= 2) {
-    regs_inc<kRegsMma>();
-    sched.init(p, BLOCK_N, 0, BK);
-    const int h = role - 1;
+  } else if (warp < 8) {
+    const int h = warp >> 2;
     const int wi = warp & 3;
     float acc[BLOCK_N / 2];
 #pragma unroll
     for (int i = 0; i < BLOCK_N / 2; ++i) acc[i] = 0.0f;
+    const int fr = h * 64 + wi * 16 + (lane >> 2), bc = 2 * (lane & 3);
+    int off[2][2];
+#pragma unroll
+    for (int e = 0; e < 2; ++e)
+#pragma unroll
+      for (int r = 0; r < 2; ++r) off[e][r] = (bc + e) * BLOCK_M + (((((fr + 8 * r) >> 2) ^ (bc + e)) << 2) | (fr & 3));
     int stage = 0; uint32_t phase = 0, tphase = 0;
     int mb, nb, kb0, kb1;
     while (sched.next(mb, nb, kb0, kb1)) {
       mma_work_item<BLOCK_N, STAGES, 0, 0, BK>(acc, p, smem, full_bar, empty_bar, h, lane, 0u, stage, phase, kb0, kb1);
-      mbar_wait(&drained_bar[h], tphase ^ 1);
-      const int r0 = h * 64 + wi * 16 + (lane >> 2), c0 = 2 * (lane & 3);
-#pragma unroll
-      for (int j = 0; j < BLOCK_N / 8; ++j) {
-        *reinterpret_cast<float2*>(&stg[r0 * SROW + 8 * j + c0]) = make_float2(acc[4 * j], acc[4 * j + 1]);
-        *reinterpret_cast<float2*>(&stg[(r0 + 8) * SROW + 8 * j + c0]) = make_float2(acc[4 * j + 2], acc[4 * j + 3]);
-      }
+      mbar_wait(&drained_bar, tphase ^ 1);
+#pragma unroll
+      for (int j = 0; j < BLOCK_N / 8; ++j)
+#pragma unroll
+        for (int e = 0; e < 2; ++e)
+#pragma unroll
+          for (int r = 0; r < 2; ++r) stg[off[e][r] + j * 8 * BLOCK_M] = acc[4 * j + 2 * r + e];
       __syncwarp();
-      if (lane == 0) mbar_arrive(&staged_bar[h]);
+      if (lane == 0) mbar_arrive(&staged_bar);
       tphase ^= 1;
     }
   } else {
-    regs_inc<kRegsEpilogue>();
-    sched.init(p, BLOCK_N, 0, BK);
-    const int h = role - 3;
-    const int ew = warp - 12;
-    const int wi = warp & 3;
-    const int quarter = h * 2 + (wi & 1);
-    const int half = wi >> 1;
-    const int row_in_tile = quarter * 32 + lane;
-    const int tid = threadIdx.x - 128 * role;
-    const int tiles_n = (p.N + BLOCK_N - 1) / BLOCK_N;
-    uint8_t* stg_hi = reinterpret_cast<uint8_t*>(&s_stage[ew][0][0][0]);
-    uint8_t* stg_lo = reinterpret_cast<uint8_t*>(&s_stage[ew][1][0][0]);
-    const int rsub = lane >> 1, csub = lane & 1;
+    const int t = threadIdx.x - 256;
+    const float* srow = stg + t * BLOCK_M;
     uint32_t tphase = 0;
     int mb, nb, kb0, kb1;
     while (sched.next(mb, nb, kb0, kb1)) {
-      const float* srow = stg + row_in_tile * SROW + half * HALF_N;
-      const int m = mb * BLOCK_M + row_in_tile;
-      const int n0 = nb * BLOCK_N + half * HALF_N;
-      int64_t pc = 0, pe = 0;
-      int c0 = 0x7fffffff, c1 = 0x7fffffff, c2 = 0x7fffffff;
-      float v0 = 0.0f, v1 = 0.0f, v2 = 0.0f;
-      float sc = 0.0f;
-      if (m < p.M) {
-        const int64_t row = p.rows ? (int64_t)p.rows[m] : (int64_t)m;
-        const int64_t rbeg = p.indptr[row];
-        const int32_t* tp = p.tile_ptr + (int64_t)m * (kParts * tiles_n + 1) + nb * kParts + half;
-        pc = rbeg + tp[0]; pe = rbeg + tp[1];
-        if (pc < pe) { c0 = p.indices[pc]; v0 = p.values[pc]; }
-        if (pc + 1 < pe) { c1 = p.indices[pc + 1]; v1 = p.values[pc + 1]; }
-        if (pc + 2 < pe) { c2 = p.indices[pc + 2]; v2 = p.values[pc + 2]; }
-        sc = (p.weight ? p.weight[m] : 1.0f) / ((float)p.stats[DAE_STAT_SUM_W] + kEps);
+      const int m = nb * BLOCK_N + t;
+      const int f0 = mb * BLOCK_M;
+      DecodeRow row;
+      row.open(p, m, mb);
+      named_bar_sync(1, 160);
+      if (t < BLOCK_M) {
+        const float b = (f0 + t < p.M) ? p.bv[f0 + t] : 0.0f;
+        s_bias[t] = b;
+        if (kFast) s_biasc[t] = b * kLog2e;
       }
-      named_bar_sync(1 + h, 128);
-      {
-        const float b = (nb * BLOCK_N + tid < p.N) ? p.bv[nb * BLOCK_N + tid] : 0.0f;
-        s_bias[h][tid] = b;
-        if (kFast) s_biasc[h][tid] = b * kLog2e;
-      }
-      mbar_wait(&staged_bar[h], tphase);
-      named_bar_sync(1 + h, 128);
-      const float inv_sc = (sc != 0.0f) ? 1.0f / sc : 0.0f;
-      const bool edge = (n0 + HALF_N > p.N);
+      mbar_wait(&staged_bar, tphase);
+      named_bar_sync(1, 160);
       float lsum = 0.0f;
-      const int m_base = mb * BLOCK_M + quarter * 32;
-      const int n_lim = edge ? p.N : 0x7fffffff;
 #pragma unroll 1
-      for (int c = 0; c < HALF_N / 16; ++c) {
+      for (int c = 0; c < BLOCK_M / 16; ++c) {
+        const int nc = f0 + 16 * c;
+        const bool edge = (f0 + 64 * (c >> 2) + 64 > p.M);
+        const int n_lim = edge ? p.M : 0x7fffffff;
         uint32_t r[16];
-        stage_ld16(srow + c * 16, r);
-        const int nc = n0 + c * 16;
-        if (m < p.M) {
-          const float* bias = &s_bias[h][half * HALF_N + c * 16];
+        stage_ld16(srow, 4 * c, t & 7, r);
+        if (m < p.N) {
+          const float* bias = &s_bias[16 * c];
           uint32_t hpk[8], lpk[8];
           bool fast_ok = false;
           if (kFast && !edge) {
             const float l0 = lsum;
-            fast_ok = decode_chunk_sigmoid_ce(r, &s_biasc[h][half * HALF_N + c * 16], sc, hpk, lpk, lsum);
-            if (!fast_ok) { lsum = l0; decode_chunk_generic<ACT, LOSS>(r, bias, sc, edge, n_lim, nc, hpk, lpk, lsum); }
+            fast_ok = decode_chunk_sigmoid_ce(r, &s_biasc[16 * c], row.sc, hpk, lpk, lsum);
+            if (!fast_ok) { lsum = l0; decode_chunk_generic<ACT, LOSS>(r, bias, row.sc, edge, n_lim, nc, hpk, lpk, lsum); }
           } else {
-            decode_chunk_generic<ACT, LOSS>(r, bias, sc, edge, n_lim, nc, hpk, lpk, lsum);
+            decode_chunk_generic<ACT, LOSS>(r, bias, row.sc, edge, n_lim, nc, hpk, lpk, lsum);
           }
-          uint4* sh = reinterpret_cast<uint4*>(stg_hi + lane * 48);
-          uint4* sl = reinterpret_cast<uint4*>(stg_lo + lane * 48);
-          sh[0] = make_uint4(hpk[0], hpk[1], hpk[2], hpk[3]); sh[1] = make_uint4(hpk[4], hpk[5], hpk[6], hpk[7]);
-          sl[0] = make_uint4(lpk[0], lpk[1], lpk[2], lpk[3]); sl[1] = make_uint4(lpk[4], lpk[5], lpk[6], lpk[7]);
-          while (c0 < nc + 16) {
-            const float x = v0;
-            const int j = c0 - nc;
-            __nv_bfloat16* ph = reinterpret_cast<__nv_bfloat16*>(stg_hi + lane * 48) + j;
-            __nv_bfloat16* pl = reinterpret_cast<__nv_bfloat16*>(stg_lo + lane * 48) + j;
+          while (row.c0 < nc + 16) {
+            const float x = row.v0;
+            const int j = row.c0 - nc;
             float d;
-            if (kFast && fast_ok && sc != 0.0f) d = (__bfloat162float(*ph) + __bfloat162float(*pl)) * inv_sc;
+            if (kFast && fast_ok && row.sc != 0.0f) d = (bf16_get16(hpk, j) + bf16_get16(lpk, j)) * (1.0f / row.sc);
             else d = act_fast<ACT>(select16(r, j) + bias[j]);
             const float gp = act_grad_from_y<ACT>(d);
             float dz;
@@ -662,38 +702,45 @@
               const float a = d + kEps, b = (1.0f - d) + kEps;
               const float la = f_lg2(a), lb = f_lg2(b);
               lsum += lb - (x * la + (1.0f - x) * lb);
-              dz = sc * gp * ((1.0f - x) * f_rcp(b) - x * f_rcp(a));
+              dz = row.sc * gp * ((1.0f - x) * f_rcp(b) - x * f_rcp(a));
             } else {
               const float e2 = x - d;
               lsum += e2 * e2 - d * d;
-              dz = -2.0f * sc * e2 * gp;
+              dz = -2.0f * row.sc * e2 * gp;
             }
             const __nv_bfloat16 hb = __float2bfloat16_rn(dz);
-            *ph = hb;
-            *pl = __float2bfloat16_rn(dz - __bfloat162float(hb));
-            ++pc;
-            c0 = c1; v0 = v1; c1 = c2; v1 = v2;
-            c2 = 0x7fffffff;
-            if (pc + 2 < pe) { c2 = p.indices[pc + 2]; v2 = p.values[pc + 2]; }
+            bf16_set16(hpk, j, __bfloat16_as_ushort(hb));
+            bf16_set16(lpk, j, __bfloat16_as_ushort(__float2bfloat16_rn(dz - __bfloat162float(hb))));
+            row.advance(p);
           }
+          uint4* slot = reinterpret_cast<uint4*>(const_cast<float*>(srow));
+          slot[(4 * c) ^ (t & 7)] = make_uint4(hpk[0], hpk[1], hpk[2], hpk[3]);
+          slot[(4 * c + 1) ^ (t & 7)] = make_uint4(hpk[4], hpk[5], hpk[6], hpk[7]);
+          slot[(4 * c + 2) ^ (t & 7)] = make_uint4(lpk[0], lpk[1], lpk[2], lpk[3]);
+          slot[(4 * c + 3) ^ (t & 7)] = make_uint4(lpk[4], lpk[5], lpk[6], lpk[7]);
         }
-        __syncwarp();
-        if (nc < p.ld_dz) {
-#pragma unroll
-          for (int i = 0; i < 2; ++i) {
-            const int rr = rsub + 16 * i;
-            if (m_base + rr < p.M) {
-              const int64_t off = (int64_t)(m_base + rr) * p.ld_dz + nc + csub * 8;
-              *reinterpret_cast<uint4*>(p.dz_hi + off) = *reinterpret_cast<const uint4*>(stg_hi + rr * 48 + csub * 16);
-              *reinterpret_cast<uint4*>(p.dz_lo + off) = *reinterpret_cast<const uint4*>(stg_lo + rr * 48 + csub * 16);
+      }
+      __syncwarp();
+      {
+        const int q = lane & 15, c = q >> 1;
+        if (f0 + 8 * q < p.ld_dz) {
+#pragma unroll 4
+          for (int i = 0; i < 16; ++i) {
+            const int rw = (t & ~31) + 2 * i + (lane >> 4);
+            const int mw = nb * BLOCK_N + rw;
+            if (mw < p.N) {
+              const uint4* sl = reinterpret_cast<const uint4*>(stg + rw * BLOCK_M);
+              const int64_t off = (int64_t)mw * p.ld_dz + f0 + 8 * q;
+              *reinterpret_cast<uint4*>(p.dz_hi + off) = sl[(4 * c + (q & 1)) ^ (rw & 7)];
+              *reinterpret_cast<uint4*>(p.dz_lo + off) = sl[(4 * c + 2 + (q & 1)) ^ (rw & 7)];
             }
           }
         }
-        __syncwarp();
       }
-      if (lane == 0) mbar_arrive(&drained_bar[h]);
+      __syncwarp();
+      if (lane == 0) mbar_arrive(&drained_bar);
       tphase ^= 1;
-      if (m < p.M) atomicAdd(p.row_loss_part + m, (LOSS == DAE_LOSS_CE) ? lsum * 0.6931471805599453f : lsum);
+      if (m < p.N) atomicAdd(p.row_loss_part + m, (LOSS == DAE_LOSS_CE) ? lsum * 0.6931471805599453f : lsum);
     }
   }
 }
@@ -703,6 +750,13 @@
 constexpr int kTopkMinTiles = 4;
 constexpr int kTopkBK = 64;
 constexpr int kTopkStages = 2;
+constexpr int kTopkN = 128;
+constexpr int kTopkThreads = 640;
+constexpr int kTopkRegsProducer = 32, kTopkRegsMma = 104, kTopkRegsEpilogue = 120;
+static_assert(128 * kTopkRegsProducer + 256 * kTopkRegsMma + 256 * kTopkRegsEpilogue <= kTopkThreads * 96, "register budget");
+
+template <int R> __device__ __forceinline__ void regs_dec() { asm volatile("setmaxnreg.dec.sync.aligned.u32 %0;" ::"n"(R)); }
+template <int R> __device__ __forceinline__ void regs_inc() { asm volatile("setmaxnreg.inc.sync.aligned.u32 %0;" ::"n"(R)); }
 
 struct TopkParams {
   GemmParams g;
@@ -763,12 +817,12 @@
 }
 
 template <int KMAX>
-__global__ void __launch_bounds__(kDecodeThreads, 1) topk_kernel(const __grid_constant__ CUtensorMap tm_a_hi,
+__global__ void __launch_bounds__(kTopkThreads, 1) topk_kernel(const __grid_constant__ CUtensorMap tm_a_hi,
                                                                  const __grid_constant__ CUtensorMap tm_a_lo,
                                                                  const __grid_constant__ CUtensorMap tm_b_hi,
                                                                  const __grid_constant__ CUtensorMap tm_b_lo,
                                                                  const TopkParams tp) {
-  constexpr int BLOCK_N = kDecodeN, STAGES = kTopkStages, BK = kTopkBK;
+  constexpr int BLOCK_N = kTopkN, STAGES = kTopkStages, BK = kTopkBK;
   constexpr int STAGE_BYTES = 2 * BLOCK_M * BK * 2 + 2 * BLOCK_N * BK * 2;
   constexpr int SROW = BLOCK_N + 4;
   constexpr int HALF_N = BLOCK_N / 2;
@@ -791,12 +845,12 @@
   __syncthreads();
 
   if (role == 0) {
-    regs_dec<kRegsProducer>();
+    regs_dec<kTopkRegsProducer>();
     sched.init(tp, BLOCK_N, BK);
     if (warp == 0 && lane == 0)
       tma_produce<BLOCK_N, STAGES, 0, BK>(p, sched, smem, full_bar, empty_bar, 0u, &tm_a_hi, &tm_a_lo, &tm_b_hi, &tm_b_lo, &tm_a_hi, &tm_a_lo);
   } else if (role <= 2) {
-    regs_inc<kRegsMma>();
+    regs_inc<kTopkRegsMma>();
     sched.init(tp, BLOCK_N, BK);
     const int h = role - 1;
     const int wi = warp & 3;
@@ -819,7 +873,7 @@
       tphase ^= 1;
     }
   } else {
-    regs_inc<kRegsEpilogue>();
+    regs_inc<kTopkRegsEpilogue>();
     sched.init(tp, BLOCK_N, BK);
     const int h = role - 3;
     const int wi = warp & 3;
@@ -1046,7 +1100,8 @@
   if ((rc = make_map(&ta_lo, A.lo, p.K, p.M, A.ld, BLOCK_M, kDecodeBK))) return rc;
   if ((rc = make_map(&tb_hi, B.hi, p.K, p.N, B.ld, kDecodeN, kDecodeBK))) return rc;
   if ((rc = make_map(&tb_lo, B.lo, p.K, p.N, B.ld, kDecodeN, kDecodeBK))) return rc;
-  constexpr int smem = kDecodeStages * (2 * BLOCK_M * kDecodeBK * 2 + 2 * kDecodeN * kDecodeBK * 2) + BLOCK_M * (kDecodeN + 4) * 4 + 1024;
+  constexpr int smem = kDecodeStages * (2 * BLOCK_M * kDecodeBK * 2 + 2 * kDecodeN * kDecodeBK * 2) + kDecodeN * BLOCK_M * 4 + 1024;
+  static_assert(smem + 2048 <= 227 * 1024, "decode shared memory");
   auto kern = decode_fused_kernel<ACT, LOSS>;
   static bool attr_done[64] = {false};
   if ((rc = ensure_smem_attr(kern, smem, attr_done))) return rc;
@@ -1063,20 +1118,20 @@
   const GemmParams& p = tp.g;
   if ((rc = make_map(&ta_hi, A.hi, p.K, p.M, A.ld, BLOCK_M, kTopkBK))) return rc;
   if ((rc = make_map(&ta_lo, A.lo, p.K, p.M, A.ld, BLOCK_M, kTopkBK))) return rc;
-  if ((rc = make_map(&tb_hi, B.hi, p.K, p.N, B.ld, kDecodeN, kTopkBK))) return rc;
-  if ((rc = make_map(&tb_lo, B.lo, p.K, p.N, B.ld, kDecodeN, kTopkBK))) return rc;
-  constexpr int smem = kTopkStages * (2 * BLOCK_M * kTopkBK * 2 + 2 * kDecodeN * kTopkBK * 2) + BLOCK_M * (kDecodeN + 4) * 4 + 1024;
+  if ((rc = make_map(&tb_hi, B.hi, p.K, p.N, B.ld, kTopkN, kTopkBK))) return rc;
+  if ((rc = make_map(&tb_lo, B.lo, p.K, p.N, B.ld, kTopkN, kTopkBK))) return rc;
+  constexpr int smem = kTopkStages * (2 * BLOCK_M * kTopkBK * 2 + 2 * kTopkN * kTopkBK * 2) + BLOCK_M * (kTopkN + 4) * 4 + 1024;
   auto kern = topk_kernel<KMAX>;
   static bool attr_done[64] = {false};
   if ((rc = ensure_smem_attr(kern, smem, attr_done))) return rc;
   const int items = ((p.M + BLOCK_M - 1) / BLOCK_M) * tp.splits;
   const int n = items < sm_count() ? items : sm_count();
-  kern<<<n, kDecodeThreads, smem, st>>>(ta_hi, ta_lo, tb_hi, tb_lo, tp);
+  kern<<<n, kTopkThreads, smem, st>>>(ta_hi, ta_lo, tb_hi, tb_lo, tp);
   return DAE_OK;
 }
 
 static int topk_splits(int n_query, int n_corpus, int requested) {
-  const int tiles_m = (n_query + BLOCK_M - 1) / BLOCK_M, tiles_n = (n_corpus + kDecodeN - 1) / kDecodeN;
+  const int tiles_m = (n_query + BLOCK_M - 1) / BLOCK_M, tiles_n = (n_corpus + kTopkN - 1) / kTopkN;
   int s = requested;
   if (s <= 0) {
     s = (sm_count() + tiles_m - 1) / tiles_m;
@@ -1193,9 +1248,9 @@
   DAE_REQUIRE(Brows > 0 && F > 0 && indptr && indices && row_loss_part && tile_ptr, "dae_decode_prepare: bad arguments");
   cudaStream_t st = (cudaStream_t)stream;
   DAE_CUDA(cudaMemsetAsync(row_loss_part, 0, sizeof(float) * Brows, st));
-  const int n_half = 2 * ((F + kDecodeN - 1) / kDecodeN);
+  const int n_half = 2 * ((F + BLOCK_M - 1) / BLOCK_M);
   dim3 grid((n_half + 1 + 127) / 128, Brows);
-  decode_tile_ptr_kernel<<<grid, 128, 0, st>>>(indptr, indices, rows, Brows, n_half, kDecodeN / 2, tile_ptr);
+  decode_tile_ptr_kernel<<<grid, 128, 0, st>>>(indptr, indices, rows, Brows, n_half, BLOCK_M / 2, tile_ptr);
   DAE_CHECK_LAUNCH("dae_decode_prepare");
   return DAE_OK;
 }
@@ -1211,7 +1266,7 @@
   DAE_REQUIRE(lde % 8 == 0 && ldw % 8 == 0 && ld_dz % 32 == 0 && ld_dz >= F, "dae_decode_fused_bf16x3: bad leading dimensions");
   cudaStream_t st = (cudaStream_t)stream;
   GemmParams p{};
-  p.M = Brows; p.N = F; p.K = K; p.k_splits = 1; p.alpha = 1.0f; p.special_col = -1;
+  p.M = F; p.N = Brows; p.K = K; p.k_splits = 1; p.alpha = 1.0f; p.special_col = -1;
   p.indptr = indptr; p.indices = indices; p.values = values; p.rows = rows; p.bv = bv; p.weight = weight; p.stats = stats;
   p.dz_hi = (__nv_bfloat16*)dz_hi; p.dz_lo = (__nv_bfloat16*)dz_lo; p.ld_dz = ld_dz; p.row_loss_part = row_loss_part;
   p.tile_ptr = tile_ptr;
@@ -1219,7 +1274,7 @@
     int rc0 = dae_decode_prepare(Brows, F, indptr, indices, rows, row_loss_part, tile_ptr, stream);
     if (rc0) return rc0;
   }
-  Operand A{e_hi, e_lo, lde, 0}, B{w_hi, w_lo, ldw, 0};
+  Operand A{w_hi, w_lo, ldw, 0}, B{e_hi, e_lo, lde, 0};
   int rc = 0;
 #define DAE_DEC(ACT, LOSS) rc = launch_decode<ACT, LOSS>(A, B, p, st)
   if (loss_func == DAE_LOSS_CE) {
```
